# taylorlu/voicepuppet

Hardware: AMD Instinct MI355X
Metric: PixReferNet G+D step frames/sec @256x256 bs=32 (higher is better)
Workload: dtype bf16; 1 GPU; PixReferNet G+D training step (G + 3xD + VGG16-conv3_3 perceptual + TF-Adam x2), 256x256, ngf=ndf=64, global batch 32 = 32 per GPU; global_batch=32, per_gpu_batch=32, parallelism=dp1

## Files before the change

voicepuppet_amd/csrc/conv_args.h:

```cpp
#pragma once
#include <stddef.h>
#include <stdint.h>

namespace vp {

struct TapTable {
  int8_t dh[16];
  int8_t dw[16];
};

struct PixSrc {
  const void* ptr[2];
  int C[2];
  const float* aff_a[2];
  const float* aff_b[2];
  int act;
  int group_n;
};

enum ConvKernel {
  CK_IGEMM = 0,
  CK_PATCH,
  CK_PATCH2,
  CK_SMALLP,
  CK_S2C64,
  CK_CIN8,
  CK_COUT8,
  CK_DCOUT8,
  CK_COUT4,
  CK_C64,
  CK_PATCH3,
  CK_PATCH4,
  CK_DC256,
  CK_DC64,
};
inline int conv_staging(int k) {
  return k <= CK_S2C64 ? k : (k <= CK_COUT4 ? CK_IGEMM : (k <= CK_PATCH4 ? CK_PATCH : CK_PATCH2));
}

struct IgemmArgs {
  PixSrc x;
  int N, Hin, Win;
  int Cin, log2Cin;
  int cin_mask;
  int cin_real;
  int Hg, Wg;
  int sh, sw;
  int ntaps, nclass;
  TapTable taps[4];
  const void* Wp;
  int Kpad, CoutPad;
  int wp_rows;
  void* Y;
  int y_f32;
  int Cout, ldY;
  int Hof, Wof, os;
  int o0h[4], o0w[4];
  const float* bias;
  int out_act;
  const void* ref;
  const float* ref_a;
  const float* ref_b;
  int ref_act, ref_group_n, accumulate;
  int split_c;
  void* Y2;
  const void* ref2;
  int accumulate2;
  int y2_f32;
  int splitk;
  float* partial;
  int vec_epi;
  int fastk;
  int rowperm;
  int xcd_remap;
  double* bn_part;
  int bn_tpg, bn_nchunk;
  const void* bst_y;
  const void* bst_y2;
  double* bn_part2;
  double* colsum_part;
  const void* zeros;
  int kern, p_kw, p_dhf, p_dhs, p_dwf, p_dws;
  void* xa_lrelu;
  void* xa_relu;
  void* pool_out;
  int pool_only;
  unsigned char* pool_code;
  int pool_src;
  unsigned* sp_cnt;
  unsigned short sp_mask[4];
  int sp_npt, sp_lcpt;
};

struct WgradArgs {
  PixSrc g;
  int Gc, log2Gc;
  int gc_mask;
  int Hgin, Wgin;
  PixSrc d;
  int Dc;
  int N, Hb, Wb;
  int s, ntaps;
  TapTable taps;
  int Mpad, Dpad;
  int splitk;
  float* partial;
  float* dW;
  int Greal, Dreal, accumulate;
  const void* zeros;
  int lw, lh;
  int fastw;
  int xcd_remap;
  int fast_tr;
};

struct Cout1Args {
  const void* dy;
  int ld_dy;
  const float* w;
  const void* ref;
  int ref_act;
  const void* y;
  double* part;
  void* dx;
  int N, H, W, C, Ho, Wo, ks, pad;
  int groups, rows;
  float* slabs;
  float* dW;
  int pix_per_group, tiles_per_group;
};

}
```

voicepuppet_amd/csrc/conv_ops.h:

```cpp
#pragma once
#include <stdlib.h>
#include <string.h>

#include "launch.h"

namespace vp {

struct ConvGeomX : ConvGeom {
  int CoutT;
};

inline ConvGeomX make_geom(int kind, int ks, int stride, int pad, int N, int Hin, int Win, int Cin, int Cin_real, int Cout) {
  ConvGeomX g;
  g.kind = kind; g.ks = ks; g.stride = stride; g.pad = pad;
  g.N = N; g.Hin = Hin; g.Win = Win;
  if (kind == 0) { g.Hout = (Hin + 2 * pad - ks) / stride + 1; g.Wout = (Win + 2 * pad - ks) / stride + 1; }
  else { g.Hout = 2 * Hin; g.Wout = 2 * Win; }
  g.Cin = Cin; g.Cin_real = Cin_real; g.Cout = Cout;
  g.CoutT = Cout < 8 ? 8 : Cout;
  return g;
}

inline int kc_elems(int is_bf16) { return is_bf16 ? 32 : 16; }

// ... 10 lines not shown
    if (rows % 128 == 0) return 0;
    if (rows % 64 == 0) return 1;
    if (rows <= 16) return 2;
    return rows > 64 ? 0 : 1;
  }
  if (rows <= 64) return 5;
  return P > 16 ? 3 : 4;
}

constexpr int IGEMM_SPLITK_TARGET_DEFAULT = 64;
inline int& igemm_splitk_target_knob() { static int v = IGEMM_SPLITK_TARGET_DEFAULT; return v; }
inline int pick_igemm_splitk(int blocks, int nchunk) {
  const int target = igemm_splitk_target_knob();
  const int cap = plan_misc_knob(1);
  const int minchunk = plan_misc_knob(2);
  if (blocks >= 256 || blocks >= target) return 1;
  int s = (target + blocks - 1) / blocks;
  if (s > nchunk / minchunk) s = nchunk / minchunk;
  if (s > cap) s = cap;
  return s < 1 ? 1 : s;
}

inline void set_single_src(PixSrc& x, const void* p, int C, const float* a, const float* b, int act, int group_n) {
  x.ptr[0] = p; x.ptr[1] = nullptr; x.C[0] = C; x.C[1] = 0;
  x.aff_a[0] = a; x.aff_b[0] = b; x.aff_a[1] = nullptr; x.aff_b[1] = nullptr;
  x.act = act; x.group_n = group_n > 0 ? group_n : (1 << 30);
}

struct LaunchForm {
  bool bias = false, ref = false, xa_lrelu = false, xa_relu = false, x_affine = false;
  bool stats = false;
  int x_act = 0, ref_act = 0;
};

struct IgemmPlan {
  IgemmArgs a;
  int cfg;
  LaunchForm form;
  PackDesc pack;
  size_t pack_elems;
  size_t partial_bytes;
};

struct IgemmPin { int cfg, splitk; };

inline void finish_igemm(IgemmPlan& p, int rows, int is_bf16, const IgemmPin* pin = nullptr) {
  IgemmArgs& a = p.a;
  const int P = a.N * a.Hg * a.Wg;
  a.Kpad = round_up(a.ntaps * a.Cin, kc_elems(is_bf16));
  p.cfg = pick_igemm_cfg(rows, P, a.Kpad);
  if (!is_bf16 && a.ntaps == 1 && p.cfg == 0) {
    const long long b128 = (long long)((P + 127) / 128) * (rows / 128), b64 = 2 * b128;
    if (((b64 + 255) / 256) * 64 < ((b128 + 255) / 256) * 128) p.cfg = 1;
  }
  if (pin) p.cfg = pin->cfg;
  int bc, bp;
  igemm_tile(p.cfg, &bc, &bp);
  a.CoutPad = round_up(rows, bc);
  if (a.ntaps == 1) { a.log2Cin = 30; a.cin_mask = 0x3fffffff; }
  else { a.log2Cin = ilog2(a.Cin); a.cin_mask = a.Cin - 1; }
  const int blocks = ((P + bp - 1) / bp) * (a.CoutPad / bc) * a.nclass;
  a.splitk = pin ? pin->splitk : pick_igemm_splitk(blocks, a.Kpad / kc_elems(is_bf16));
  p.partial_bytes = a.splitk > 1 ? (size_t)a.nclass * a.splitk * P * a.CoutPad * sizeof(float) : 0;
  {
    const bool tc4 = p.cfg == 0 || p.cfg == 1 || p.cfg == 6 || p.cfg == 7 || p.cfg == 8 || p.cfg == 9;
    a.rowperm = (tc4 && rows % 64 == 0) ? 1 : 0;
    p.pack.perm = a.rowperm;
  }
  a.wp_rows = round_up(rows, 128);
  p.pack.rows_pad = a.wp_rows;
  p.pack.Kpad = a.Kpad;
  p.pack.kc = kc_elems(is_bf16);
  p.pack_elems = (size_t)a.nclass * a.wp_rows * a.Kpad;
}

inline int& patch_tiles_knob() { static int v = 7; return v; }
inline int& patch_small_knob() { static int v = 3; return v; }
inline int& patch_longk_knob() { static int v = 1; return v; }
inline int& patch3_knob() { static int v = 1; return v; }
inline int& wgrad_big_knob() { static int v = 1; return v; }
inline int& patch4_knob() { static int v = 1; return v; }
inline int& c64_knob() { static int v = 1; return v; }
inline int& pool_bwd_fused_knob() { static int v = 1; return v; }
inline int& cout1_knob() { static int v = 256; return v; }
inline int& wgrad1_rows_knob() { static int v = 512; return v; }
inline int& dc64_knob() { static int v = 1; return v; }
inline int& s2c64_knob() { static int v = 512; return v; }
inline int& s2c64_pair_knob() { static int v = 1; return v; }
constexpr int PATCH_MIN_BLOCKS_DEFAULT = 192;
inline int& patch_minblk_knob() { static int v = PATCH_MIN_BLOCKS_DEFAULT; return v; }

inline void patch_tile_hw(int bp, int* th, int* tw) { *th = bp == 128 ? 8 : 16; *tw = bp == 512 ? 32 : 16; }
inline int patch_tile_pixels(int bc) {
  const int k = patch_small_knob();
  if (bc == 256) return (k & 2) ? 128 : 256;
  return (k & 1) ? 256 : 512;
}

inline int patch_tile_rows(int rows, int on) {
  if ((on & 1) && rows % 256 == 0) return 256;
  if ((on & 2) && rows % 128 == 0) return 128;
  if ((on & 4) && rows % 64 == 0) return 64;
  return 0;
}

inline bool plan_patch_eligible(const IgemmPlan& p, int rows, int is_bf16, bool single_src, bool any_grid = false) {
  const int on = patch_tiles_knob();
  const int minblk = any_grid ? 0 : patch_minblk_knob();
  const IgemmArgs& a = p.a;
  const int kc = kc_elems(is_bf16);
  if (!on || !single_src || a.nclass != 1 || a.sh != 1 || a.sw != 1 || a.os != 1 || a.ntaps < 9 || a.Cin % kc || a.Cin < kc) return false;
  if (rows % 64 || a.Cout % 8 || a.ldY % 8 || a.Hg < 16 || a.Wg < 16 || a.Hof != a.Hg || a.Wof != a.Wg) return false;
  const bool p4 = patch4_knob() && is_bf16 && a.ntaps == 16 && rows % 128 == 0;
  if (!p4 && patch_longk_knob() && rows >= 512 && rows % 256 == 0 && a.ntaps * a.Cin >= 4096 && (long long)a.N * a.Hg * a.Wg >= 256 * 256) return false;
  const int bc = p4 ? 128 : patch_tile_rows(rows, on);
  if (!bc) return false;
  int th, tw;
  patch_tile_hw(p4 ? 256 : patch_tile_pixels(bc), &th, &tw);
  const long long blocks = (long long)a.N * ((a.Hg + th - 1) / th) * ((a.Wg + tw - 1) / tw) * (rows / bc);
  const long long p4min = (long long)a.ntaps * a.Cin >= 8192 ? 256 : 512;
  if (p4 && !any_grid && patch_minblk_knob() > 1) {
    if (blocks < p4min) return false;
  } else if (blocks < minblk) return false;
  if ((size_t)a.N * a.Hin * a.Win * a.Cin * (is_bf16 ? 2 : 4) >= 0x70000000ull) return false;
  int ks = 0;
  while (ks * ks < a.ntaps) ++ks;
  if (ks * ks != a.ntaps) return false;
  const int sh = a.taps[0].dh[ks] - a.taps[0].dh[0], sw = a.taps[0].dw[1] - a.taps[0].dw[0];
  if ((sh != 1 && sh != -1) || (sw != 1 && sw != -1)) return false;
  for (int t = 0; t < a.ntaps; ++t)
    if (a.taps[0].dh[t] != a.taps[0].dh[0] + (t / ks) * sh || a.taps[0].dw[t] != a.taps[0].dw[0] + (t % ks) * sw) return false;
  return true;
}
inline void plan_make_patch(IgemmPlan& p, int rows, int is_bf16) {
  IgemmArgs& a = p.a;
  const bool p4 = patch4_knob() && is_bf16 && a.ntaps == 16 && rows % 128 == 0;
  const int bc = p4 ? 128 : patch_tile_rows(rows, patch_tiles_knob());
  int ks = 0;
  while (ks * ks < a.ntaps) ++ks;
  a.kern = CK_PATCH; a.p_kw = ks;
  a.p_dhf = a.taps[0].dh[0]; a.p_dwf = a.taps[0].dw[0];
  a.p_dhs = a.taps[0].dh[ks] - a.taps[0].dh[0]; a.p_dws = a.taps[0].dw[1] - a.taps[0].dw[0];
  const int bp = p4 ? 256 : patch_tile_pixels(bc);
  p.cfg = bc == 256 ? (bp == 128 ? 15 : 10) : (bc == 128 ? (bp == 256 ? 13 : 11) : (bp == 256 ? 14 : 12));
  a.CoutPad = round_up(rows, bc);
  a.splitk = 1;
  p.partial_bytes = 0;
  a.rowperm = 1;
  p.pack.perm = 1;
  p.pack.kswap = 1;
}

inline int& patch_xcd_knob() { static int v = 0; return v; }
inline int& patch2_knob() { static int v = 1; return v; }
inline bool plan_patch2_eligible(const IgemmPlan& p, int rows, int is_bf16, int c0, int c1) {
  const IgemmArgs& a = p.a;
  const int kc = kc_elems(is_bf16);
  if (!patch2_knob() || a.nclass != 4 || a.ntaps != 4 || a.os != 2 || a.sh != 1 || a.sw != 1) return false;
  if (c0 + c1 != a.Cin || c0 % (2 * kc) || c1 % (2 * kc) || c0 < 2 * kc) return false;
  if (rows % 64 || rows > 128 || a.Cout % 8 || a.ldY % 8 || a.Hg < 16 || a.Wg < 16 || a.Hof != 2 * a.Hg || a.Wof != 2 * a.Wg) return false;
  const long long blocks = (long long)a.N * ((a.Hg + 15) / 16) * ((a.Wg + 15) / 16) * 4;
  if (blocks < patch_minblk_knob()) return false;
  const size_t cmax = c0 > c1 ? c0 : c1;
  if ((size_t)a.N * a.Hin * a.Win * cmax * (is_bf16 ? 2 : 4) >= 0x70000000ull) return false;
  for (int cls = 0; cls < 4; ++cls)
    for (int t = 0; t < 4; ++t)
// ... 281 lines not shown
```

voicepuppet_amd/csrc/conv_patch3.hip:

```cpp
#include <stdlib.h>
#ifndef VP_P3_NO_NT
#define VP_NT_STORE 1
#endif
#ifndef VP_P3_ABL
#define VP_P3_ABL 0
#endif

#include <utility>

#include "conv_ops.h"
#include "igemm_device.h"
#include "launch.h"
#include "patch_device.h"

namespace vp {

template <typename T, int WC, int WP, int TC, int TP, int TH, int TW, int NSTW, int KW>
using Patch3Geom = PatchGeom<T, WC, WP, TC, TP, TH, TW, KW - 1, NSTW>;

template <typename T, int WC, int WP, int TC, int TP, int TH, int TW, int STATS, int OCC, int NSTW = 3, int KW = 3>
__global__ __launch_bounds__(512, OCC) void igemm_patch3_kernel(const IgemmArgs a) {
  using G = Patch3Geom<T, WC, WP, TC, TP, TH, TW, NSTW, KW>;
  constexpr int E = G::E, KC = G::KC, NW = G::NW, LA = NSTW - 1;
  constexpr int KS2 = KW * KW, TRIP = 2 * KS2;
  static_assert(TRIP % NSTW == 0 && NSTW >= 3, "ring stages");
  constexpr int JA = G::JA, PW = G::PW, JP = G::JP, PBUFB = G::PBUFB, WSTB = G::WSTB, WBASE = G::WBASE;
  static_assert(JP + LA <= KS2, "one patch DMA per tap step, none in the last LA steps of a chunk");
  extern __shared__ __attribute__((aligned(16))) char smem[];

  const int tid = threadIdx.x, lane = tid & 63;
  const int wave = __builtin_amdgcn_readfirstlane(tid >> 6);
  const int c_base = blockIdx.y * G::BC;
  const PatchTile tile = patch_tile_origin<TH, TW>(a, a.xcd_remap);
  const int n = tile.n, y0 = tile.y0, x0 = tile.x0;
  const bool flip = a.p_dhs < 0;
  const int dh0 = flip ? a.p_dhf - (KW - 1) : a.p_dhf, dw0 = flip ? a.p_dwf - (KW - 1) : a.p_dwf;
  const unsigned es = sizeof(T);
  const int C0 = a.x.C[0];
  const int nchunkc = C0 / KC;

  __amdgpu_buffer_rsrc_t rsW = make_rsrc(reinterpret_cast<const T*>(a.Wp), 0xFFFFFFFFu);
  __amdgpu_buffer_rsrc_t rsX = make_rsrc(a.x.ptr[0], (unsigned)((size_t)a.N * a.Hin * a.Win * C0 * es));

  unsigned pvo[JP];
#pragma unroll
  for (int j = 0; j < JP; ++j) {
    const int pp = (wave + NW * j) * 16 + (lane >> 2);
    const int py = pp / PW, px = pp - py * PW;
    const int ih = y0 + dh0 + py, iw = x0 + dw0 + px;
    const bool ok = pp < G::NPATCH && (unsigned)ih < (unsigned)a.Hin && (unsigned)iw < (unsigned)a.Win;
    const int piece = (lane & 3) ^ ((px >> 2) & 3);
    pvo[j] = ok ? (unsigned)((((n * a.Hin + ih) * a.Win + iw) * C0 + piece * E) * es) : DMA_OOB;
  }
  const PatchWeightDma<G> wdma(c_base, wave, lane);
  const unsigned wstep = (unsigned)(a.wp_rows * KC * es);
  auto issue_w = [&](int u, int chunk, int stage) {
    const int tap = flip ? KS2 - 1 - u : u;
    wdma.issue(rsW, (unsigned)(tap * nchunkc + chunk) * wstep, reinterpret_cast<uint4*>(smem + WBASE + stage * WSTB));
  };
  auto issue_p = [&](int chunk, int buf, int j) {
    uint4* lb = reinterpret_cast<uint4*>(smem + buf * PBUFB);
    dma16_buf(rsX, pvo[j], (unsigned)(chunk * KC) * es, lb + (wave + NW * j) * 64);
  };

  const int wc = wave / WP, wpi = wave - wc * WP;
  const int blkA0 = wc * TC, blkB0 = wpi * TP;
  const int fi = lane & 15, fg = lane >> 4;
  const int aaddr = WBASE + (blkA0 * 64 + fi * 4 + (fg ^ rb_swz(fi))) * 16;
  int tb0[KW][TP];
#pragma unroll
  for (int c = 0; c < KW; ++c)
#pragma unroll
    for (int q = 0; q < TP; ++q) {
      constexpr int BPR = TW / 16;
      const int pb = blkB0 + q;
      const int px = (pb % BPR) * 16 + fi + c;
      const int pp = (pb / BPR) * PW + px;
      tb0[c][q] = (pp << 6) + (((fg ^ (px >> 2)) & 3) << 4) + ((fg & 1) << 3);
    }

  f32x4 acc[TC][TP];
#pragma unroll
  for (int i = 0; i < TC; ++i)
#pragma unroll
    for (int j = 0; j < TP; ++j) acc[i][j] = (f32x4){0.f, 0.f, 0.f, 0.f};

#pragma unroll
  for (int j = 0; j < JP; ++j) issue_p(0, 0, j);
#pragma unroll
  for (int d = 0; d < LA; ++d) issue_w(d % KS2, d / KS2, d % NSTW);

  for (int c = 0; c < ((VP_P3_ABL & 16) ? 0 : nchunkc); c += 2) {
    const bool last_pair = c + 2 >= nchunkc;
    auto step = [&](auto uc) {
      constexpr int U = decltype(uc)::value;
      constexpr int cc = U / KS2, u = U % KS2, pr = u / KW, pc = u % KW, stage = U % NSTW;
      constexpr int NPIECE = [] { int n = 0; for (int k = 1; k <= LA; ++k) n += ((U + TRIP - k) % TRIP % KS2) < JP ? 1 : 0; return n; }();
      constexpr int NV = (LA - 1) * JA + NPIECE;
      constexpr int WLAST = (TRIP - 1 - U < LA - 1 ? TRIP - 1 - U : LA - 1);
#if !(VP_P3_ABL & 2)
      if (U + LA - 1 > TRIP - 1 && last_pair) wait_vm<WLAST * JA + NPIECE>();
      else wait_vm<NV>();
#endif
#if !(VP_P3_ABL & 1)
      __builtin_amdgcn_s_barrier();
#endif
      asm volatile("" ::: "memory");
#if !(VP_P3_ABL & 4)
      {
        constexpr int UL = (U + LA) % TRIP;
        if (U + LA < TRIP) issue_w(UL % KS2, c + UL / KS2, (U + LA) % NSTW);
        else if (!last_pair) issue_w(UL % KS2, c + 2 + UL / KS2, (U + LA) % NSTW);
      }
      if constexpr (u < JP) issue_p(c + cc + 1, 1 - cc, u);
#endif
      constexpr int NA = TC == 8 ? 4 : ((TC == 4 && OCC == 4) ? 2 : TC);
      patch_step_mma<T, TC, TP, NA, stage * WSTB, cc * PBUFB + pr * PW * 64, true>(aaddr, tb0[pc], acc);
    };
    static_steps(step, std::make_integer_sequence<int, TRIP>{});
  }
  asm volatile("s_waitcnt vmcnt(0)" ::: "memory");

#ifndef VP_P3_NO_FASTEPI
  constexpr int NPASS16 = G::BC == 64 ? epi_passes16(G::BC, G::BP, WP, G::RINGB) : 0;
#else
  constexpr int NPASS16 = 0;
#endif
  if (!(VP_P3_ABL & 8) || acc[0][0][0] == 1.2345f) staged_epilogue<T, TC, TP, G::BC, G::BP, G::NPASS, G::NT, STATS, NPASS16>(a, PatchTilePix<TW>{a, n, y0, x0}, c_base, blkA0, blkB0, acc, smem, tile.bt, 0);
}

template <typename T, int WC, int WP, int TC, int TP, int TH, int TW, int OCC, int NSTW = 3, int KW = 3>
static hipError_t launch_patch3_t(const IgemmArgs& b, hipStream_t st) {
  auto kern = b.bn_part ? igemm_patch3_kernel<T, WC, WP, TC, TP, TH, TW, 1, OCC, NSTW, KW> : igemm_patch3_kernel<T, WC, WP, TC, TP, TH, TW, 0, OCC, NSTW, KW>;
  if (b.bst_y) {
    if constexpr (KW == 4) kern = igemm_patch3_kernel<T, WC, WP, TC, TP, TH, TW, 2, OCC, NSTW, KW>;
    else return hipErrorInvalidValue;
  }
  return launch_patch_grid<Patch3Geom<T, WC, WP, TC, TP, TH, TW, NSTW, KW>>(kern, b, 1, st);
}

bool patch3_eligible(const IgemmArgs& a, int is_bf16) {
  const int kc = is_bf16 ? 32 : 16;
  return conv_staging(a.kern) == CK_PATCH && a.ntaps == 9 && a.p_kw == 3 && a.p_dhs == a.p_dws && (a.p_dhs == 1 || a.p_dhs == -1) && a.x.C[0] % (2 * kc) == 0 &&
         a.x.C[1] == 0;
}

bool patch4_eligible(const IgemmArgs& a, int is_bf16) {
  return is_bf16 && conv_staging(a.kern) == CK_PATCH && a.ntaps == 16 && a.p_kw == 4 && a.p_dhs == a.p_dws && (a.p_dhs == 1 || a.p_dhs == -1) &&
         a.x.C[0] % 64 == 0 && a.x.C[1] == 0 && a.CoutPad % 128 == 0 && !a.pool_out;
}
hipError_t launch_igemm_patch4(const IgemmArgs& a, hipStream_t st) {
  IgemmArgs b = a;
  b.vec_epi = 1;
  b.xcd_remap = patch_xcd_knob();
  return launch_patch3_t<bf16, 2, 4, 4, 4, 16, 16, 4, 4, 4>(b, st);
}

hipError_t launch_igemm_patch3(const IgemmArgs& a, int is_bf16, int bc, int bp, hipStream_t st) {
  IgemmArgs b = a;
  b.vec_epi = 1;
  b.xcd_remap = patch_xcd_knob();
#define VP_PATCH3_GO(WC, WP, TC, TP, TH, TW, OCC) \
  (is_bf16 ? launch_patch3_t<bf16, WC, WP, TC, TP, TH, TW, OCC>(b, st) : launch_patch3_t<float, WC, WP, TC, TP, TH, TW, OCC>(b, st))
#define VP_PATCH3_GO6(WC, WP, TC, TP, TH, TW, OCC) \
  (is_bf16 ? launch_patch3_t<bf16, WC, WP, TC, TP, TH, TW, OCC, 6>(b, st) : launch_patch3_t<float, WC, WP, TC, TP, TH, TW, OCC, 6>(b, st))
  if (bc == 256) return bp == 128 ? VP_PATCH3_GO(2, 4, 8, 2, 8, 16, 4) : VP_PATCH3_GO(2, 4, 8, 4, 16, 16, 2);
  if (bc == 128) return bp == 512 ? VP_PATCH3_GO(1, 8, 8, 4, 16, 32, 2) : VP_PATCH3_GO(2, 4, 4, 4, 16, 16, 4);
  if (bp == 512) return VP_PATCH3_GO(1, 8, 4, 4, 16, 32, 2);
  return VP_PATCH3_GO6(2, 4, 2, 4, 16, 16, 4);
#undef VP_PATCH3_GO6
#undef VP_PATCH3_GO
}

}
```

voicepuppet_amd/csrc/igemm_device.h:

```cpp
#pragma once
#include "conv_args.h"
#include "vp_common.h"

namespace vp {

__device__ __forceinline__ int rb_swz(int i) { return (0x78 >> ((i >> 1) & 6)) & 3; }

template <typename T, int TC, int TP, int BC, int BP>
__device__ __forceinline__ void mma_chunk_rb(const uint4* __restrict__ ldsA, const uint4* __restrict__ ldsB,
                                             int blkA0, int blkB0, int lane, f32x4 (&acc)[TC][TP]) {
  const int i = lane & 15, g = lane >> 4;
  const int so = i * 4 + (g ^ rb_swz(i));
  uint4 fa[TC], fb[TP];
#pragma unroll
  for (int t = 0; t < TC; ++t) fa[t] = ldsA[(blkA0 + t) * 64 + so];
#pragma unroll
  for (int t = 0; t < TP; ++t) fb[t] = ldsB[(blkB0 + t) * 64 + so];
#pragma unroll
  for (int tc = 0; tc < TC; ++tc)
#pragma unroll
    for (int tp = 0; tp < TP; ++tp) acc[tc][tp] = mma16<T>(fa[tc], fb[tp], acc[tc][tp]);
}

__device__ __forceinline__ void dma16(const void* src, uint4* lds_dst_wave_uniform) {
// ... 31 lines not shown
}

constexpr int epi_passes16(int BC, int BP, int WP, int ring_bytes) {
  for (int np = 1; np <= WP; np *= 2)
    if ((BP / np) * (BC * 2 + 16) + (BP / np) * 8 <= ring_bytes) return np;
  return WP;
}

template <typename T, bool DUAL = false>
__device__ __forceinline__ void epi_store8(const IgemmArgs& a, long long ot, int c0, size_t off, float (&v)[8]) {
  void* Yp = a.Y;
  const void* refp = a.ref;
  int accu = a.accumulate, yf32 = a.y_f32;
  if constexpr (DUAL) {
    if (c0 >= a.split_c) {
      Yp = a.Y2; refp = a.ref2; accu = a.accumulate2; yf32 = a.y2_f32;
      c0 -= a.split_c; off -= (size_t)a.split_c;
    }
  }
  if (a.bias) {
#pragma unroll
    for (int e = 0; e < 8; ++e) v[e] += a.bias[c0 + e];
  }
  if (a.out_act != ACT_NONE) {
#pragma unroll
    for (int e = 0; e < 8; ++e) v[e] = act_apply(a.out_act, v[e]);
  }
  if (refp) {
    float z[8];
    const T* rp = reinterpret_cast<const T*>(refp) + off;
    if (sizeof(T) == 2) Elem<bf16>::unpack(*reinterpret_cast<const uint4*>(rp), z);
    else {
      Elem<float>::unpack(reinterpret_cast<const uint4*>(rp)[0], z);
      Elem<float>::unpack(reinterpret_cast<const uint4*>(rp)[1], z + 4);
    }
    if (a.ref_a) {
      const int goff = (int)(ot & 255) * a.Cout + c0;
#pragma unroll
      for (int e = 0; e < 8; ++e) z[e] = fmaf(a.ref_a[goff + e], z[e], a.ref_b[goff + e]);
    }
#pragma unroll
    for (int e = 0; e < 8; ++e) v[e] *= act_grad(a.ref_act, z[e]);
  }
  if (yf32 || sizeof(T) == 4) {
    float* yp = reinterpret_cast<float*>(Yp) + off;
    if (accu) {
      const float4 e0 = reinterpret_cast<const float4*>(yp)[0], e1 = reinterpret_cast<const float4*>(yp)[1];
      v[0] += e0.x; v[1] += e0.y; v[2] += e0.z; v[3] += e0.w; v[4] += e1.x; v[5] += e1.y; v[6] += e1.z; v[7] += e1.w;
    }
#ifdef VP_NT_STORE
#pragma unroll
    for (int e = 0; e < 8; ++e) __builtin_nontemporal_store(v[e], yp + e);
#else
    reinterpret_cast<float4*>(yp)[0] = make_float4(v[0], v[1], v[2], v[3]);
    reinterpret_cast<float4*>(yp)[1] = make_float4(v[4], v[5], v[6], v[7]);
#endif
  } else {
    bf16* yp = reinterpret_cast<bf16*>(Yp) + off;
    if (accu) {
      float e[8];
      Elem<bf16>::unpack(*reinterpret_cast<const uint4*>(yp), e);
#pragma unroll
      for (int k = 0; k < 8; ++k) v[k] += e[k];
    }
#ifdef VP_NT_STORE
    { const uint4 pk = Elem<bf16>::pack(v); __builtin_nontemporal_store(pk.x, reinterpret_cast<unsigned*>(yp)); __builtin_nontemporal_store(pk.y, reinterpret_cast<unsigned*>(yp) + 1);
      __builtin_nontemporal_store(pk.z, reinterpret_cast<unsigned*>(yp) + 2); __builtin_nontemporal_store(pk.w, reinterpret_cast<unsigned*>(yp) + 3); }
#else
    *reinterpret_cast<uint4*>(yp) = Elem<bf16>::pack(v);
#endif
  }
}


__device__ __forceinline__ unsigned pool_code_of(float v0, float v1, float v2, float v3) {
  unsigned best = 0;
  float m = v0;
  if (v1 > m) { m = v1; best = 1; }
  if (v2 > m) { m = v2; best = 2; }
  if (v3 > m) { m = v3; best = 3; }
  return m > 0.f ? 1u + best : 0u;
}

template <typename T, int TC, int TP, int BC, int BP, int NPASS, int NT, int STATS = 0, int NPASS16 = 0, bool DUAL = false, typename PixFn>
__device__ __forceinline__ void staged_epilogue(const IgemmArgs& a, const PixFn& pixfn, int c_base, int blkA0, int blkB0,
                                                f32x4 (&acc)[TC][TP], char* smem, int pt = 0, int cls = 0) {
  if constexpr (NPASS16 > 0 && sizeof(T) == 2 && STATS == 0) {
    if (!a.ref && !a.accumulate && !a.y_f32 && (a.out_act == ACT_NONE || a.out_act == ACT_RELU)) {
      constexpr int PITCHB = BC * 2 + 16, CGB = BC / 8, RPB = BP / NPASS16;
      static_assert(RPB % (TP * 16) == 0, "a wave's pixel rows must fall into one pass");
      const int tid = threadIdx.x, lane = tid & 63;
      long long* otab = reinterpret_cast<long long*>(smem + RPB * PITCHB);
#pragma unroll
      for (int ps = 0; ps < NPASS16; ++ps) {
        __syncthreads();
        if (tid < RPB) otab[tid] = pixfn(ps * RPB + tid);
        if (blkB0 * 16 >= ps * RPB && blkB0 * 16 < (ps + 1) * RPB) {
#pragma unroll
          for (int tc = 0; tc < TC; ++tc) {
            const int ch = tile_chan0(a.rowperm, blkA0 + tc, lane >> 4);
            float b4[4] = {0.f, 0.f, 0.f, 0.f};
            if (a.bias && c_base + ch < a.Cout) {
#pragma unroll
              for (int e = 0; e < 4; ++e) b4[e] = a.bias[c_base + ch + e];
            }
#pragma unroll
            for (int tp = 0; tp < TP; ++tp) {
              const int row = (blkB0 + tp) * 16 + (lane & 15) - ps * RPB;
              float v[4];
#pragma unroll
              for (int e = 0; e < 4; ++e) {
                v[e] = acc[tc][tp][e];
                if (a.bias) v[e] += b4[e];
                if (a.out_act != ACT_NONE) v[e] = act_apply(a.out_act, v[e]);
              }
              uint2 pk;
              pk.x = Elem<bf16>::pack2(v[0], v[1]); pk.y = Elem<bf16>::pack2(v[2], v[3]);
              *reinterpret_cast<uint2*>(smem + row * PITCHB + ch * 2) = pk;
            }
            __builtin_amdgcn_sched_barrier(0);
          }
        }
        __syncthreads();
        bool store_y = true;
        if constexpr (pix_has_pool<PixFn>::value) store_y = !(a.pool_out != nullptr && a.pool_only);
        if (store_y)
          for (int idx = tid; idx < RPB * CGB; idx += NT) {
            const int p = idx / CGB, cgp = idx - p * CGB;
            const long long ot = otab[p];
            const int c0 = c_base + cgp * 8;
            if (ot < 0 || c0 >= a.Cout) continue;
            const uint4 pk = *reinterpret_cast<const uint4*>(smem + p * PITCHB + cgp * 16);
            unsigned* yp = reinterpret_cast<unsigned*>(reinterpret_cast<bf16*>(a.Y) + (size_t)(ot >> 8) + c0);
#ifdef VP_NT_STORE
            __builtin_nontemporal_store(pk.x, yp); __builtin_nontemporal_store(pk.y, yp + 1);
            __builtin_nontemporal_store(pk.z, yp + 2); __builtin_nontemporal_store(pk.w, yp + 3);
#else
            *reinterpret_cast<uint4*>(yp) = pk;
#endif
          }
        if constexpr (pix_has_pool<PixFn>::value) {
          if (a.pool_out != nullptr) {
            static_assert(RPB % 32 == 0, "a pass must hold whole pairs of tile rows");
            constexpr int PR = RPB / 4;
            for (int idx = tid; idx < PR * CGB; idx += NT) {
              const int pp = idx / CGB, cgp = idx - pp * CGB;
              const int pyl = pp >> 3, pxl = pp & 7;
              const int c0 = c_base + cgp * 8;
              const long long po = pixfn.pool(ps * (RPB / 32) + pyl, pxl);
              if (po < 0 || c0 >= a.Cout) continue;
              const int r00 = pyl * 32 + pxl * 2;
              float m[8];
#pragma unroll
              for (int k = 0; k < 4; ++k) {
                const int rr = r00 + (k >> 1) * 16 + (k & 1);
                float v[8];
                Elem<bf16>::unpack(*reinterpret_cast<const uint4*>(smem + rr * PITCHB + cgp * 16), v);
#pragma unroll
                for (int e = 0; e < 8; ++e) m[e] = k == 0 ? v[e] : fmaxf(m[e], v[e]);
              }
              *reinterpret_cast<uint4*>(reinterpret_cast<bf16*>(a.pool_out) + po + c0) = Elem<bf16>::pack(m);
              if (a.pool_code) {
                float vv[4][8];
#pragma unroll
                for (int k = 0; k < 4; ++k)
                  Elem<bf16>::unpack(*reinterpret_cast<const uint4*>(smem + (r00 + (k >> 1) * 16 + (k & 1)) * PITCHB + cgp * 16), vv[k]);
                unsigned w[2] = {0u, 0u};
#pragma unroll
                for (int e = 0; e < 8; ++e) w[e >> 2] |= pool_code_of(vv[0][e], vv[1][e], vv[2][e], vv[3][e]) << (8 * (e & 3));
                *reinterpret_cast<uint2*>(a.pool_code + po + c0) = make_uint2(w[0], w[1]);
              }
            }
          }
        }
      }
      return;
    }
  }
  constexpr int PITCH = BC * 4 + 16;
  constexpr int CG = BC / 8;
  constexpr int RP = BP / NPASS;
  static_assert(RP % (TP * 16) == 0, "a wave's pixel rows must fall into one pass");
  const int tid = threadIdx.x, lane = tid & 63;
  long long* otab = reinterpret_cast<long long*>(smem + RP * PITCH);
  static_assert(STATS != 1 || NT % BC == 0, "column sums: whole thread groups per channel");
  static_assert(STATS != 2 || NT % CG == 0, "backward sums: a thread keeps one channel group");
  float bsum = 0.f, bsq = 0.f;
  float gs0[STATS == 2 ? 8 : 1], gs1[STATS == 2 ? 8 : 1];
  const T* gy = nullptr;
  if constexpr (STATS == 2) {
    int c0 = c_base + (tid % CG) * 8;
    const void* yb = a.bst_y;
    int ct = a.Cout;
    if constexpr (DUAL) {
      ct = a.split_c;
      if (c0 >= a.split_c) { yb = a.bst_y2; c0 -= a.split_c; }
    }
#pragma unroll
    for (int e = 0; e < 8; ++e) { gs0[e] = 0.f; gs1[e] = 0.f; }
    if (yb && c0 < ct) gy = reinterpret_cast<const T*>(yb);
  }
#pragma unroll
  for (int ps = 0; ps < NPASS; ++ps) {
    __syncthreads();
    if (tid < RP) otab[tid] = pixfn(ps * RP + tid);
    if (blkB0 * 16 >= ps * RP && blkB0 * 16 < (ps + 1) * RP) {
#pragma unroll
      for (int tp = 0; tp < TP; ++tp)
#pragma unroll
        for (int tc = 0; tc < TC; ++tc) {
          const int row = (blkB0 + tp) * 16 + (lane & 15) - ps * RP;
          const int ch = tile_chan0(a.rowperm, blkA0 + tc, lane >> 4);
          *reinterpret_cast<f32x4*>(smem + row * PITCH + ch * 4) = acc[tc][tp];
          __builtin_amdgcn_sched_barrier(0);
        }
    }
    __syncthreads();
    if constexpr (STATS == 1) {
      const int col = tid % BC;
      for (int rr = tid / BC; rr < RP; rr += NT / BC) {
        if (otab[rr] < 0) continue;
        float x = *reinterpret_cast<const float*>(smem + rr * PITCH + col * 4);
        if (sizeof(T) == 2) x = bf16_bits_to_f32(f32_to_bf16_bits(x));
        bsum += x; bsq = fmaf(x, x, bsq);
      }
    }
    bool store_y = true;
    if constexpr (pix_has_pool<PixFn>::value) store_y = !(a.pool_out != nullptr && a.pool_only);
    if (store_y)
    for (int idx = tid; idx < RP * CG; idx += NT) {
      const int p = idx / CG, cgp = idx - p * CG;
      const long long ot = otab[p];
      const int c0 = c_base + cgp * 8;
      if (ot < 0 || c0 >= a.Cout) continue;
      const size_t off = (size_t)(ot >> 8) + c0;
      float v[8];
      {
        const float4 v0 = *reinterpret_cast<const float4*>(smem + p * PITCH + cgp * 32);
        const float4 v1 = *reinterpret_cast<const float4*>(smem + p * PITCH + cgp * 32 + 16);
        v[0] = v0.x; v[1] = v0.y; v[2] = v0.z; v[3] = v0.w; v[4] = v1.x; v[5] = v1.y; v[6] = v1.z; v[7] = v1.w;
      }
      uint4 ry0 = make_uint4(0, 0, 0, 0), ry1 = make_uint4(0, 0, 0, 0);
      if constexpr (STATS == 2) {
        if (gy) {
          size_t yo = off;
          if constexpr (DUAL) { if (c0 >= a.split_c) yo -= (size_t)a.split_c; }
          ry0 = reinterpret_cast<const uint4*>(gy + yo)[0];
          if (sizeof(T) == 4) ry1 = reinterpret_cast<const uint4*>(gy + yo)[1];
        }
      }
      epi_store8<T, DUAL>(a, ot, c0, off, v);
      if constexpr (STATS == 2) {
        if (gy) {
          float fy[8];
          if (sizeof(T) == 2) Elem<bf16>::unpack(ry0, fy);
          else { Elem<float>::unpack(ry0, fy); Elem<float>::unpack(ry1, fy + 4); }
// ... 112 lines not shown
```

voicepuppet_amd/csrc/launch.h:

```cpp
#pragma once
#include <hip/hip_runtime.h>

#include "conv_args.h"
#include "pointwise_args.h"

namespace vp {

hipError_t launch_igemm(const IgemmArgs& a, int is_bf16, int cfg, hipStream_t st);
void igemm_tile(int cfg, int* bc, int* bp);
hipError_t launch_igemm_patch(const IgemmArgs& a, int is_bf16, int bc, int bp, hipStream_t st);
bool patch3_eligible(const IgemmArgs& a, int is_bf16);
hipError_t launch_igemm_patch3(const IgemmArgs& a, int is_bf16, int bc, int bp, hipStream_t st);
bool patch4_eligible(const IgemmArgs& a, int is_bf16);
hipError_t launch_igemm_patch4(const IgemmArgs& a, hipStream_t st);
bool conv_kernel_ok(const IgemmArgs& a, int is_bf16);
const char* conv_kernel_name(int kern);
bool conv_cin8_eligible(const IgemmArgs& a, int is_bf16);
hipError_t launch_conv_cin8(const IgemmArgs& a, hipStream_t st);
bool conv_cout8_eligible(const IgemmArgs& a, int is_bf16);
hipError_t launch_conv_cout8(const IgemmArgs& a, hipStream_t st);
bool conv_dcout8_eligible(const IgemmArgs& a, int is_bf16);
hipError_t launch_conv_dcout8(const IgemmArgs& a, hipStream_t st);
bool conv_cout4_eligible(const IgemmArgs& a, int is_bf16);
hipError_t launch_conv_cout4(const IgemmArgs& a, hipStream_t st);
bool conv_c64_eligible(const IgemmArgs& a, int is_bf16);
hipError_t launch_conv_c64(const IgemmArgs& a, hipStream_t st);
bool conv_dc64_eligible(const IgemmArgs& a, int is_bf16);
hipError_t launch_conv_dc64(const IgemmArgs& a, hipStream_t st);
int conv_dc64_grid(const IgemmArgs& a);
bool conv_dc256_eligible(const IgemmArgs& a, int is_bf16);
int conv_dc256_grid(const IgemmArgs& a);
hipError_t launch_conv_dc256(const IgemmArgs& a, hipStream_t st);
bool conv_s2c64_eligible(const IgemmArgs& a, int is_bf16);
int conv_s2c64_grid(const IgemmArgs& a);
int conv_s2c64_tiles_per_image(const IgemmArgs& a);
hipError_t launch_conv_s2c64(const IgemmArgs& a, hipStream_t st);
bool conv_cout1_bwd_eligible(const Cout1Args& a);
hipError_t launch_conv_cout1_bwd(const Cout1Args& a, hipStream_t st);
bool conv_cout1_wgrad_eligible(const Cout1Args& a);
hipError_t launch_conv_cout1_wgrad(const Cout1Args& a, hipStream_t st);
hipError_t launch_cout1_wgrad_prof(const Cout1Args& a, hipStream_t st);
hipError_t launch_cout1_bwd_prof(const Cout1Args& a, hipStream_t st);
hipError_t launch_igemm_patch2(const IgemmArgs& a, int is_bf16, int bc, int bp, hipStream_t st);
hipError_t launch_igemm_smallp(const IgemmArgs& a, int is_bf16, hipStream_t st);
struct SmallPArgs;
hipError_t launch_smallp(const SmallPArgs& s, int is_bf16, hipStream_t st);
hipError_t launch_smallp_fused(const SmallPArgs& s, int is_bf16, hipStream_t st);
hipError_t launch_wgrad(const WgradArgs& a, int is_bf16, int cfg, hipStream_t st);
bool wgrad_mm_eligible(const WgradArgs& a, int cfg);
hipError_t launch_wgrad_mm(const WgradArgs& a, int cfg, hipStream_t st);
hipError_t launch_wgrad_tr(const WgradArgs& a, hipStream_t st, const char** variant = nullptr, int* tile_cols = nullptr);
void wgrad_tile(int cfg, int* bm, int* bn);

void profile_enable(int on);
void profile_tag(const char* tag);
size_t profile_collect(char* out, size_t cap);

hipError_t launch_pack_weights(const PackDesc* d_descs, int ndesc, const float* master, void* packed, int is_bf16, hipStream_t st);
hipError_t launch_pack_weights_one(const PackDesc& d, const float* master, void* packed, int is_bf16, hipStream_t st);
int bn_nchunk(int Pg, int C, int G, int is_bf16);
hipError_t launch_bn_stats(const BnArgs& a, int is_bf16, hipStream_t st);
hipError_t launch_bn_finalize(const BnArgs& a, hipStream_t st);
bool bn_small(const BnArgs& a);
hipError_t launch_bn_small_fwd(const BnArgs& a, void* out_lrelu, void* out_relu, int is_bf16, hipStream_t st);
hipError_t launch_bn_small_bwd(const BnArgs& a, int is_bf16, hipStream_t st);
hipError_t launch_bn_bwd(const BnArgs& a, int is_bf16, hipStream_t st);
hipError_t launch_bn_bwd_tail(const BnArgs& a, int is_bf16, hipStream_t st);
hipError_t launch_colsum(const BnArgs& a, int creal, float* out, int accumulate, int is_bf16, hipStream_t st);
hipError_t launch_colsum_tail(const BnArgs& a, int creal, float* out, int accumulate, hipStream_t st);
hipError_t launch_act_apply(const void* y, const float* sc, const float* sh, int C, int Pg, size_t npix,
                            void* out_lrelu, void* out_relu, int is_bf16, hipStream_t st);
hipError_t launch_tap_gather(const TapArgs& a, hipStream_t st);
hipError_t launch_tap_spread(const TapArgs& a, int is_bf16, hipStream_t st);
hipError_t launch_frame_pack(const FramePackArgs& a, hipStream_t st);
hipError_t launch_pack_inputs(const PackInputsArgs& a, int is_bf16, hipStream_t st);
int composite_nblocks(int N, int HW);
hipError_t launch_composite_fwd(const CompositeArgs& a, int is_bf16, hipStream_t st);
hipError_t launch_composite_bwd(const CompositeArgs& a, int is_bf16, hipStream_t st);
hipError_t launch_gan_loss(const GanLossArgs& a, int is_bf16, hipStream_t st);
int perceptual_nblocks(size_t half, int is_bf16);
hipError_t launch_perceptual(const PerceptualArgs& a, int is_bf16, hipStream_t st);
hipError_t launch_loss_final(const LossFinalArgs& a, hipStream_t st);
hipError_t launch_maxpool_fwd(const void* x, void* y, int B, int H, int W, int C, int is_bf16, hipStream_t st);
hipError_t launch_maxpool_bwd(const void* x, const void* dy, void* dx, int B, int H, int W, int C, int is_bf16, hipStream_t st);
hipError_t launch_maxpool_bwd_code(const void* code, const void* dy, void* dx, int B, int H, int W, int C, int is_bf16, hipStream_t st);
hipError_t launch_relu_bwd(const void* y, void* d, size_t n, int is_bf16, hipStream_t st);
hipError_t launch_adam(const AdamArgs& a, hipStream_t st);
hipError_t launch_fetch(const FetchArgs& a, hipStream_t st);
hipError_t launch_grad_pack_bf16(const float* src, void* dst, size_t n, hipStream_t st);
hipError_t launch_grad_unpack_bf16(const void* src, float* dst, size_t n, float scale, hipStream_t st);

struct ConvGeom {
  int kind;
  int ks, stride, pad;
  int N, Hin, Win, Hout, Wout;
  int Cin, Cin_real;
  int Cout;
};

inline int ilog2(int v) { int l = 0; while ((1 << l) < v) ++l; return l; }
inline int round_up(int v, int m) { return (v + m - 1) / m * m; }

}
```

voicepuppet_amd/csrc/ops_api.hip:

```cpp
#include <string.h>

#include <string>

#include "conv_ops.h"
#include "errors.h"
#include "audio_args.h"
#include "launch.h"
#include "vp_common.h"

using namespace vp;

namespace {

bool conv_desc_ok(const vp_conv_desc* d) {
  if (!d || d->n < 1 || d->h < 1 || d->w < 1) return false;
  if (d->cin < 8 || (d->cin & (d->cin - 1))) return false;
  if (d->kind == 1 && (d->ksize != 4 || d->stride != 2 || d->pad != 1)) return false;
  if (d->kind != 0 && d->kind != 1) return false;
  if (d->ksize < 1 || d->ksize > 4 || d->stride < 1 || d->stride > 2) return false;
  if (d->kind == 0 && d->stride == 2 && (d->ksize != 4 || d->pad != 1 || (d->h & 1) || (d->w & 1))) return false;
  return d->dtype == VP_F32 || d->dtype == VP_BF16;
}

ConvGeomX geom_of(const vp_conv_desc* d) {
  return make_geom(d->kind, d->ksize, d->stride, d->pad, d->n, d->h, d->w, d->cin, d->cin, d->cout);
}

size_t align256(size_t v) { return (v + 255) & ~(size_t)255; }

const void* zero_page(char* ws, size_t used, hipStream_t st) {
  char* z = ws + align256(used);
  (void)hipMemsetAsync(z, 0, 256, st);
  return z;
}

}

extern "C" {

int vp_pixrefer_pack_frames(const unsigned char* example_frames, const unsigned char* current_frames, const int* crops,
                            int n, int img_size, float* inputs, float* fg_inputs, float* targets, float* masks, void* stream) {
  if (!example_frames || !current_frames || !crops || !inputs || !fg_inputs || !targets || !masks || n < 1 || img_size < 2) {
    set_err("vp_pixrefer_pack_frames: bad argument");
    return VP_ERR_ARG;
  }
  FramePackArgs a;
  a.ex = example_frames; a.cur = current_frames; a.crops = crops;
  a.inputs = inputs; a.fg_inputs = fg_inputs; a.targets = targets; a.masks = masks;
  a.N = n; a.S = img_size;
  VP_HIP_CHECK(launch_frame_pack(a, (hipStream_t)stream));
  return VP_OK;
}

extern "C" void vp_phase_marks_enable(int on);

int vp_tune(const char* key, int value) {
  if (!key) return VP_ERR_ARG;
  const std::string k(key);
  if (k == "patch_tiles") { patch_tiles_knob() = value; return VP_OK; }
  if (k == "patch_min_blocks") { patch_minblk_knob() = value < 0 ? PATCH_MIN_BLOCKS_DEFAULT : value; return VP_OK; }
  if (k == "patch_small_tiles") { patch_small_knob() = value; return VP_OK; }
  if (k == "patch_long_k_on_256") { patch_longk_knob() = value; return VP_OK; }
  if (k == "wgrad_tr") { wgrad_tr_knob() = value; return VP_OK; }
  if (k == "patch3") { patch3_knob() = value; return VP_OK; }
  if (k == "c64") { c64_knob() = value; return VP_OK; }
  if (k == "dc64") { dc64_knob() = value; return VP_OK; }
  if (k == "pool_bwd_fused") { pool_bwd_fused_knob() = value < 0 || value > 4 ? 1 : value; return VP_OK; }
  if (k == "cout1_wgrad_rows" && value > 0) { wgrad1_rows_knob() = value; return VP_OK; }
  if (k == "cout1_bwd") { cout1_knob() = value < 0 ? 256 : value; return VP_OK; }
  if (k == "s2c64") { s2c64_knob() = value; return VP_OK; }
  if (k == "wgrad_big") { wgrad_big_knob() = value; return VP_OK; }
  if (k == "patch4") { patch4_knob() = value; return VP_OK; }
  if (k == "s2c64_pair") { s2c64_pair_knob() = value; return VP_OK; }
  if (k == "bfm_dwproj") { bfm_dwproj_knob() = value; return VP_OK; }
  if (k == "patch2") { patch2_knob() = value; return VP_OK; }
  if (k == "patch_xcd") { patch_xcd_knob() = value; return VP_OK; }
  if (k == "smallp_max_pixels") { smallp_knob() = value; return VP_OK; }
  if (k == "igemm_splitk_target") { igemm_splitk_target_knob() = value < 0 ? IGEMM_SPLITK_TARGET_DEFAULT : value; return VP_OK; }
  if (k == "wgrad_fixed_x10") { wgrad_cost_knob(0) = value; return VP_OK; }
  if (k == "wgrad_slab_tile_x1000") { wgrad_cost_knob(2) = value < 0 ? 150 : value; return VP_OK; }
  if (k == "wgrad_slab_x100") { wgrad_cost_knob(1) = value; return VP_OK; }
  if (k == "smallp_split_target") { plan_misc_knob(0) = value; return VP_OK; }
  if (k == "igemm_splitk_cap") { plan_misc_knob(1) = value; return VP_OK; }
  if (k == "igemm_splitk_minchunk") { plan_misc_knob(2) = value; return VP_OK; }
  if (k == "wgrad_resident_blocks") { plan_misc_knob(3) = value; return VP_OK; }
  if (k == "igemm_small_grid") { igemm_small_grid_knob() = value; return VP_OK; }
  if (k == "thin_blocks_cout8" && value > 0) { thin_blocks_knob(0) = value; return VP_OK; }
  if (k == "thin_blocks_dcout8" && value > 0) { thin_blocks_knob(1) = value; return VP_OK; }
  if (k == "thin_blocks_cout4" && value > 0) { thin_blocks_knob(2) = value; return VP_OK; }
  if (k == "thin_blocks_cin8" && value > 0) { thin_blocks_knob(3) = value; return VP_OK; }
  if (k == "phase_marks") { vp_phase_marks_enable(value); return VP_OK; }
  set_err("vp_tune: unknown key %s", key);
  return VP_ERR_ARG;
}

static unsigned* smallp_counter_page(char* ws, size_t used, const IgemmArgs& a, hipStream_t st) {
  unsigned* c = (unsigned*)(ws + align256(used) + 256);
  (void)hipMemsetAsync(c, 0, (size_t)smallp_counters(a) * sizeof(unsigned), st);
  return c;
}

size_t vp_conv_workspace_bytes(const vp_conv_desc* d) {
  if (!conv_desc_ok(d)) return 0;
  const int bf = d->dtype == VP_BF16, es = bf ? 2 : 4;
  const ConvGeomX g = geom_of(d);
  size_t best = 0;
  {
    IgemmPlan p = plan_fwd(g, 0, bf);
    best = align256(p.pack_elems * es) + p.partial_bytes;
    plan_kernel(p, g.Cout, bf, d->cin, 0, FAM_SMALLP, LaunchForm{});
    if (p.a.kern == CK_SMALLP) {
      const size_t b = align256(p.pack_elems * es) + align256(p.partial_bytes) + 512 + (size_t)smallp_counters(p.a) * sizeof(unsigned);
      if (b > best) best = b;
    }
  }
  if ((d->cout & (d->cout - 1)) == 0 && d->cout >= 8) {
    IgemmPlan p = plan_bwd_data(g, 0, 0, d->cin, d->cin, d->cin, bf);
    size_t b = align256(p.pack_elems * es) + p.partial_bytes;
    if (b > best) best = b;
    plan_kernel(p, d->cin, bf, d->cout, 0, FAM_SMALLP, LaunchForm{});
    if (p.a.kern == CK_SMALLP) {
      b = align256(p.pack_elems * es) + align256(p.partial_bytes) + 512 + (size_t)smallp_counters(p.a) * sizeof(unsigned);
      if (b > best) best = b;
    }
    for (int plain = 0; plain < 2; ++plain) {
      WgradPlan w = plan_wgrad(g, bf, plain != 0);
      if (w.partial_bytes + 512 > best) best = w.partial_bytes + 512;
    }
  }
  return best + 1024;
}

int vp_conv_fwd(const vp_conv_desc* d, const void* x, const float* in_scale, const float* in_shift,
                const float* w, const float* bias, void* y, void* workspace, void* stream) {
  if (!conv_desc_ok(d) || !x || !w || !y || !workspace) { set_err("vp_conv_fwd: bad argument"); return VP_ERR_ARG; }
  const int bf = d->dtype == VP_BF16, es = bf ? 2 : 4;
  hipStream_t st = (hipStream_t)stream;
  const ConvGeomX g = geom_of(d);
  IgemmPlan p = plan_fwd(g, 0, bf);
  p.a.out_act = d->out_act;
  LaunchForm f;
  f.bias = bias != nullptr; f.x_affine = in_scale != nullptr; f.x_act = d->in_act;
  const bool plain = d->in_act == ACT_NONE && !in_scale;
  plan_kernel(p, g.Cout, bf, d->cin, 0, plain ? (FAM_SMALLP | FAM_PATCH | FAM_PATCH2 | (d->out_act == ACT_NONE ? FAM_S2C64 : 0)) : 0, f);
  char* ws = (char*)workspace;
  VP_HIP_CHECK(launch_pack_weights_one(p.pack, w, ws, bf, st));
  IgemmArgs a = p.a;
  set_single_src(a.x, x, d->cin, in_scale, in_shift, d->in_act, 0);
  a.Wp = ws;
  a.partial = (float*)(ws + align256(p.pack_elems * es));
// ... 93 lines not shown
  if (pixels < 1 || c < 8) return 0;
  const int nch = bn_nchunk(pixels, c, 1, dtype == VP_BF16);
  return (size_t)nch * 2 * c * sizeof(double) + 4 * (size_t)c * sizeof(float) + 1024;
}

static bool bn_ok(int pixels, int c, int dtype) {
  const int e = dtype == VP_BF16 ? 8 : 4;
  return pixels >= 1 && c >= e && c % e == 0 && 256 % (c / e) == 0 && (dtype == VP_F32 || dtype == VP_BF16);
}

int vp_bn_stats(const void* y, int pixels, int c, int dtype, const float* gamma, const float* beta, float eps,
                float* scale, float* shift, float* mean, float* rstd, void* workspace, void* stream) {
  if (!bn_ok(pixels, c, dtype) || !y || !gamma || !beta || !scale || !shift || !mean || !rstd || !workspace) {
    set_err("vp_bn_stats: bad argument");
    return VP_ERR_ARG;
  }
  BnArgs b;
  memset(&b, 0, sizeof(b));
  b.y = y; b.C = c; b.G = 1; b.Pg = pixels;
  b.nchunk = bn_nchunk(pixels, c, 1, dtype == VP_BF16);
  b.partial = (double*)workspace;
  b.gamma = gamma; b.beta = beta; b.aff_a = scale; b.aff_b = shift; b.mu = mean; b.rstd = rstd; b.eps = eps;
  VP_HIP_CHECK(launch_bn_stats(b, dtype == VP_BF16, (hipStream_t)stream));
  return VP_OK;
}

int vp_bn_bwd(const void* y, const void* dz, void* dy, int pixels, int c, int dtype, const float* gamma,
              const float* mean, const float* rstd, float* dgamma, float* dbeta, void* workspace, void* stream) {
  if (!bn_ok(pixels, c, dtype) || !y || !dz || !dy || !gamma || !mean || !rstd || !dgamma || !dbeta || !workspace) {
    set_err("vp_bn_bwd: bad argument");
    return VP_ERR_ARG;
  }
  BnArgs b;
  memset(&b, 0, sizeof(b));
  b.y = y; b.dz = dz; b.dy = dy; b.C = c; b.G = 1; b.Pg = pixels;
  b.nchunk = bn_nchunk(pixels, c, 1, dtype == VP_BF16);
  b.partial = (double*)workspace;
  float* f = (float*)((char*)workspace + (size_t)b.nchunk * 2 * c * sizeof(double));
  b.c1 = f; b.c2 = f + c;
  b.gamma = gamma; b.mu = const_cast<float*>(mean); b.rstd = const_cast<float*>(rstd);
  b.dgamma = dgamma; b.dbeta = dbeta;
  VP_HIP_CHECK(launch_bn_bwd(b, dtype == VP_BF16, (hipStream_t)stream));
  return VP_OK;
}


int vp_maxpool2x2_fwd(const void* x, void* y, int n, int h, int w, int c, int dtype, void* stream) {
  const int e = dtype == VP_BF16 ? 8 : 4;
  if (!x || !y || n < 1 || h < 2 || w < 2 || (h & 1) || (w & 1) || c < e || c % e) { set_err("vp_maxpool2x2_fwd: bad argument"); return VP_ERR_ARG; }
  VP_HIP_CHECK(launch_maxpool_fwd(x, y, n, h, w, c, dtype == VP_BF16, (hipStream_t)stream));
  return VP_OK;
}

int vp_maxpool2x2_bwd(const void* x, const void* dy, void* dx, int n, int h, int w, int c, int dtype, void* stream) {
  const int e = dtype == VP_BF16 ? 8 : 4;
  if (!x || !dy || !dx || n < 1 || h < 2 || w < 2 || (h & 1) || (w & 1) || c < e || c % e) { set_err("vp_maxpool2x2_bwd: bad argument"); return VP_ERR_ARG; }
  VP_HIP_CHECK(launch_maxpool_bwd(x, dy, dx, n, h, w, c, dtype == VP_BF16, (hipStream_t)stream));
  return VP_OK;
}

int vp_maxpool2x2_bwd_code(const void* code, const void* dy, void* dx, int n, int h, int w, int c, int dtype, void* stream) {
  const int e = dtype == VP_BF16 ? 8 : 4;
  if (!code || !dy || !dx || n < 1 || h < 2 || w < 2 || (h & 1) || (w & 1) || c < e || c % e) { set_err("vp_maxpool2x2_bwd_code: bad argument"); return VP_ERR_ARG; }
  VP_HIP_CHECK(launch_maxpool_bwd_code(code, dy, dx, n, h, w, c, dtype == VP_BF16, (hipStream_t)stream));
  return VP_OK;
}

int vp_composite_fwd(const float* gen_out4, const float* targets, float* out4, float* outputs, float* outputs_fg, int n, int hw,
                     void* stream) {
  if (!gen_out4 || !targets || !out4 || !outputs || !outputs_fg || n < 1 || hw < 1) { set_err("vp_composite_fwd: bad argument"); return VP_ERR_ARG; }
  CompositeArgs ca;
  memset(&ca, 0, sizeof(ca));
  ca.y4 = gen_out4; ca.targets = targets; ca.o4 = out4; ca.outputs = outputs; ca.outputs_fg = outputs_fg; ca.N = n; ca.HW = hw; ca.train = 0;
  VP_HIP_CHECK(launch_composite_fwd(ca, 0, (hipStream_t)stream));
  return VP_OK;
}

int vp_gan_loss(const float* logits, void* seed_d, void* seed_g, float* predict, float* losses, int m, float gan_weight, int dtype,
                void* stream) {
  if (!logits || !seed_d || !seed_g || !predict || !losses || m < 1) { set_err("vp_gan_loss: bad argument"); return VP_ERR_ARG; }
  GanLossArgs ga;
  memset(&ga, 0, sizeof(ga));
  ga.logits = logits; ga.dl_d = seed_d; ga.dl_g = seed_g; ga.predict = predict; ga.losses = losses; ga.M = m; ga.gan_weight = gan_weight;
  VP_HIP_CHECK(launch_gan_loss(ga, dtype == VP_BF16, (hipStream_t)stream));
  return VP_OK;
}

int vp_dwconv7x3_bn_act(const float* x, const float* w, const float* bias, float* y, int b, int h, int wd, int c, void* stream) {
  if (!x || !w || !bias || !y || b < 1 || h < 1 || wd < 1 || c < 4 || (c & 3)) { set_err("vp_dwconv7x3_bn_act: bad argument"); return VP_ERR_ARG; }
  VP_HIP_CHECK(launch_dwconv7x3(x, w, bias, y, 0, b, h, wd, c, (hipStream_t)stream));
  return VP_OK;
}

int vp_dwconv7x3_bn_act_t(const void* x, const float* w, const float* bias, void* y, int dtype, int b, int h, int wd, int c, void* stream) {
  if (!x || !w || !bias || !y || b < 1 || h < 1 || wd < 1 || c < 4 || (c & 3) || (dtype != VP_F32 && dtype != VP_BF16)) {
    set_err("vp_dwconv7x3_bn_act_t: bad argument"); return VP_ERR_ARG;
  }
  VP_HIP_CHECK(launch_dwconv7x3(x, w, bias, y, dtype == VP_BF16, b, h, wd, c, (hipStream_t)stream));
  return VP_OK;
}

int vp_conv_first_fwd(const float* x, const float* w, const float* bias, float* y, int b, int h, int w_in, int cout, void* stream) {
  if (!x || !w || !bias || !y || b < 1 || h < 1 || w_in < 1 || cout < 1) { set_err("vp_conv_first_fwd: bad argument"); return VP_ERR_ARG; }
  int pt, ho, pl, wo;
  same_pad(h, 9, 1, &pt, &ho);
  same_pad(w_in, 5, 2, &pl, &wo);
  VP_HIP_CHECK(launch_conv_first(x, w, bias, y, 0, b, h, w_in, wo, cout, pt, pl, (hipStream_t)stream));
  return VP_OK;
}

static IgemmPlan dwproj_pack_plan(int pixels, int ce, int cout) {
  IgemmPlan p = plan_fwd(make_geom(0, 1, 1, 0, 1, pixels, 1, ce, ce, cout), 0, 0);
  p.pack.s_ch = cout;
  p.pack.dst_off = 0;
  p.pack.perm = 0; p.a.rowperm = 0;
  return p;
}

size_t vp_dwproj_workspace_bytes(int ce, int cout) {
  if (ce < 16 || ce % 16 || cout < 1) return 0;
  return align256((size_t)22 * ce * sizeof(float)) + align256(dwproj_pack_plan(1, ce, cout).pack_elems * sizeof(float)) + 256;
}

int vp_dwproj_fwd(const float* ex, const float* w_dw, const float* b_dw, const float* w_proj, const float* b_proj, float* y, int add, int b, int h,
                  int w, int ce, int cout, void* workspace, void* stream) {
  if (!ex || !w_dw || !b_dw || !w_proj || !b_proj || !y || !workspace || b < 1 || h < 1 || w < 1) { set_err("vp_dwproj_fwd: bad argument"); return VP_ERR_ARG; }
  if (!dwproj_eligible(w, ce, cout)) {
    set_err("vp_dwproj_fwd: no kernel for mel width %d, %d expanded and %d output channels (dwproj_eligible)", w, ce, cout);
    return VP_ERR_ARG;
  }
  const size_t ex_bytes = (size_t)b * h * w * ce * sizeof(float);
  if (ex_bytes >= 0xF0000000ull) {
    set_err("vp_dwproj_fwd: the expanded tensor is %zu bytes, the kernel's 32-bit lane offsets stop below 0xF0000000 (%llu)", ex_bytes, 0xF0000000ull);
    return VP_ERR_ARG;
  }
  hipStream_t st = (hipStream_t)stream;
  float* wdw22 = (float*)workspace;
  float* packed = (float*)((char*)workspace + align256((size_t)22 * ce * sizeof(float)));
  VP_HIP_CHECK(hipMemcpyAsync(wdw22, w_dw, (size_t)21 * ce * sizeof(float), hipMemcpyDeviceToDevice, st));
  VP_HIP_CHECK(hipMemcpyAsync(wdw22 + (size_t)21 * ce, b_dw, (size_t)ce * sizeof(float), hipMemcpyDeviceToDevice, st));
  const IgemmPlan p = dwproj_pack_plan(b * h * w, ce, cout);
  VP_HIP_CHECK(launch_pack_weights_one(p.pack, w_proj, packed, 0, st));
  VP_HIP_CHECK(launch_dwproj(ex, wdw22, packed, p.a.wp_rows, b_proj, y, add ? 1 : 0, b, h, w, ce, cout, st));
  return VP_OK;
}

int vp_maxpool_hw(const float* x, float* y, int b, int h, int w, int c, int kh, int kw, int sh, int sw, void* stream) {
  if (!x || !y || b < 1 || h < 1 || w < 1 || c < 4 || (c & 3) || kh < 1 || kw < 1 || sh < 1 || sw < 1) { set_err("vp_maxpool_hw: bad argument"); return VP_ERR_ARG; }
  const int ho = (h + sh - 1) / sh, wo = (w + sw - 1) / sw;
  const int ph = (ho - 1) * sh + kh - h, pw = (wo - 1) * sw + kw - w;
  const int pt = ph > 0 ? ph / 2 : 0, pl = pw > 0 ? pw / 2 : 0;
  VP_HIP_CHECK(launch_maxpool_same(x, y, 0, 0, b, h, w, c, kh, kw, sh, sw, pt, pl, ho, wo, (hipStream_t)stream));
  return VP_OK;
}

int vp_gru_seq(const float* xg, const float* xc, const float* whg, const float* whc, const int* seq_len, float* out, int b, int t,
               void* stream) {
  if (!xg || !xc || !whg || !whc || !seq_len || !out || b < 1 || t < 1) { set_err("vp_gru_seq: bad argument"); return VP_ERR_ARG; }
  VP_HIP_CHECK(launch_gru_seq(xg, xc, whg, whc, seq_len, out, b, t, (hipStream_t)stream));
  return VP_OK;
}

int vp_gru_seq_state(const float* xg, const float* xc, const float* whg, const float* whc, float* hstate, float* out, int b, int t, int t0,
                     int n, void* stream) {
  if (!xg || !xc || !whg || !whc || !hstate || !out || b < 1 || t < 1 || t0 < 0 || n < 0 || t0 + n > t) {
    set_err("vp_gru_seq_state: bad argument"); return VP_ERR_ARG;
  }
// ... 16 lines not shown
```

voicepuppet_amd/csrc/plan_pixrefer.hip:

```cpp
#include <math.h>
#include <stdio.h>
#include <string.h>

#include <mutex>
#include <string>
#include <utility>
#include <vector>

#include "conv_ops.h"
#include "errors.h"
#include "launch.h"
#include "smallp_args.h"
#include "vp_common.h"

namespace vp {

thread_local char g_err[512] = "";
void set_err(const char* fmt, ...) {
  va_list ap;
  va_start(ap, fmt);
  vsnprintf(g_err, sizeof(g_err), fmt, ap);
  va_end(ap);
}

struct Arena {
  char* base;
  size_t off, cap;
  std::vector<std::pair<size_t, size_t>>* track = nullptr;
  void* alloc(size_t bytes) {
    off = (off + 255) & ~(size_t)255;
    void* p = base ? base + off : nullptr;
    if (track) track->push_back({off, bytes});
    off += bytes;
    return p;
  }
};

struct BnBuf {
  float *a, *b, *mu, *rstd, *c1, *c2, *c1g, *c2g;
  double *pb, *pbg;
};

struct Tens {
  std::string name;
  void* y = nullptr;
  void* dz = nullptr;
  int N = 0, H = 0, W = 0, C = 0;
  bool is_f32 = false;
  bool has_bn = false;
  bool is_input = false;
  bool dz_written = false;
  void* dz2 = nullptr;
  bool dz2_written = false;
  void* xa[3] = {nullptr, nullptr, nullptr};
  bool need_act[3] = {false, false, false};
  BnBuf bn{};
  int producer = -1;
  int n_bwd_consumers = 0;
  int dz_writes = 0;
  bool bn_bwd_done = false;
  bool hi = false;
  void* dz32 = nullptr;
  double* cs_part = nullptr;
  int cs_chunks = 0;
  int pb_cap = 0, pbg_cap = 0;
  int bst_chunks = 0, bst_chunks_g = 0;
  size_t elems() const { return (size_t)N * H * W * C; }
};

struct Layer {
  std::string scope;
  ConvGeomX g;
  int src[2] = {-1, -1};
  int nsrc = 1;
  int in_act = ACT_NONE;
  int out_act = ACT_NONE;
  int out = -1;
  bool has_bn = false;
  size_t w_off = 0, b_off = 0, gamma_off = 0, beta_off = 0;
  size_t pk_fwd = 0, pk_bwd[2] = {0, 0}, pk_bwd_alt[2] = {0, 0};
  bool need_bwd[2] = {false, false};
  IgemmPlan fwd, bwd[2], bwd_alt[2];
  IgemmPlan bwd_pair;
  size_t pk_bwd_pair = 0;
  bool has_pair = false;
  IgemmPlan fwd_half;
  size_t pk_fwd_half = 0;
  bool has_fwd_half = false;
  WgradPlan wg;
  size_t desc0 = 0, desc1 = 0;
  bool tapgemm = false;
  bool fwd_stats = false;
  float* tap_S = nullptr;
  void* tap_dyS = nullptr;
  unsigned* sp_cnt_fwd = nullptr;
  unsigned* sp_cnt_bwd[2] = {nullptr, nullptr};
  unsigned* sp_cnt_pair = nullptr;
};

struct ParamInfo { std::string name; size_t off; int ndim; int64_t shape[4]; };

struct Net {
  std::vector<Tens> t;
  std::vector<Layer> l;
  std::vector<ParamInfo> manifest;
  size_t nparams = 0;
  int batch = 0, groups = 1;
  float* params = nullptr;
  float* grads = nullptr;
  char* packed = nullptr;
  size_t packed_elems = 0;
  std::vector<PackDesc> descs;
  PackDesc* d_descs = nullptr;
  unsigned* sp_cnt = nullptr;
  size_t sp_cnt_n = 0;
};

}

using namespace vp;

struct vp_pixrefer {
  vp_pixrefer_desc d;
  int bf16, es;
  Net G, D, V;
  void *gin, *gfg, *din, *vin;
  float *y4, *o4, *outputs, *outputs_fg, *logits, *predict, *losses;
  void *dl_d, *dl_g, *d_din, *d_vin, *dy4, *df3;
  void *vpool1, *vpool2, *d_vpool1, *d_vpool2;
  unsigned char* vpool_code[2];
  bool pool_codes_written;
  bool pool_fuse_ok[2];
  bool pool_bwd_fused;
  bool pool_dz_stale[2];
  double *comp_partial, *perc_partial, *bn_partial;
  char* scratch;
  char* scratch2;
  double* bn_partial2;
  char* scratch3;
  double* bn_partial3;
  char* scratch4;
  double* bn_partial4;
  hipStream_t side, branch;
  hipStream_t branch2;
  hipEvent_t ev_b2join;
  bool use_b2;
  hipEvent_t ev_fork, ev_join, ev_bfork, ev_bjoin;
  hipEvent_t ev_upd_b, ev_upd_m;
  bool overlap, forked;
  int bst_count;
  int bst_on;
  int vgg_fork_layer;
  bool store_first_raw;
  bool ov_on;
  int dfork_point;
  bool dsplit_on;
  hipEvent_t mark[64];
  int nmark;
  bool marks_made;
  int dfork_pending;
  void* zeros;
  size_t scratch_bytes;
  int n_comp, n_perc;
  struct { bool active, d_done; float *m_g, *v_g, *m_d, *v_d; float lr_t_g, lr_t_d, beta1, beta2, eps; } upd;
  int upd_mask;
  bool params_dirty;
  bool vgg_dirty;
  const float *in_targets, *in_masks;
};

namespace vp {

static int add_tensor(Net& n, const std::string& name, int N, int H, int W, int C, bool has_bn, bool is_input) {
  Tens t;
  t.name = name; t.N = N; t.H = H; t.W = W; t.C = C; t.has_bn = has_bn; t.is_input = is_input;
  n.t.push_back(t);
  return (int)n.t.size() - 1;
}

static void add_param(Net& n, const std::string& name, std::initializer_list<int64_t> shape, size_t* off_out) {
  ParamInfo p;
  p.name = name; p.off = n.nparams; p.ndim = (int)shape.size();
  size_t cnt = 1;
  int i = 0;
  for (auto s : shape) { p.shape[i++] = s; cnt *= (size_t)s; }
  for (; i < 4; ++i) p.shape[i] = 1;
  *off_out = n.nparams;
  n.nparams += cnt;
  n.manifest.push_back(p);
}

static int add_layer(Net& n, const std::string& prefix, const std::string& scope, int kind, int ks, int stride, int pad,
                     std::initializer_list<int> srcs, int cin_real, int cout, bool has_bn, int in_act, int out_act,
                     const char* wname, const char* bname) {
  Layer L;
  L.scope = scope;
  L.nsrc = 0;
  int cin = 0;
  for (int s : srcs) {
    L.src[L.nsrc++] = s; cin += n.t[s].C;
    if (in_act != ACT_NONE) n.t[s].need_act[in_act] = true;
  }
  const Tens& t0 = n.t[L.src[0]];
  L.g = make_geom(kind, ks, stride, pad, n.batch, t0.H, t0.W, cin, cin_real, cout);
  L.in_act = in_act; L.out_act = out_act; L.has_bn = has_bn;
  const std::string base = prefix + scope + "/";
  if (kind == 0) add_param(n, base + wname, {ks, ks, cin_real, cout}, &L.w_off);
  else add_param(n, base + wname, {4, 4, cout, cin_real}, &L.w_off);
  add_param(n, base + bname, {cout}, &L.b_off);
  if (has_bn) {
    add_param(n, base + "batch_normalization/gamma", {cout}, &L.gamma_off);
    add_param(n, base + "batch_normalization/beta", {cout}, &L.beta_off);
  }
  L.out = add_tensor(n, scope, n.batch, L.g.Hout, L.g.Wout, L.g.CoutT, has_bn, false);
  n.t[L.out].producer = (int)n.l.size();
  n.l.push_back(L);
  return L.out;
}
// ... 233 lines not shown
    if (training && L.has_pair && L.bwd_pair.a.kern == CK_SMALLP) n.sp_cnt_n += smallp_counters(L.bwd_pair.a);
  }
}

static void carve_net(Net& n, Arena& ar, int es, bool training) {
  for (Tens& t : n.t) {
    if (t.name == "decoder_1" || t.name == "layer_5") {
      continue;
    }
    if (!t.is_input) t.y = ar.alloc(t.elems() * (t.hi ? sizeof(float) : (size_t)es));
    for (int k = 1; k < 3; ++k) if (t.need_act[k]) t.xa[k] = ar.alloc(t.elems() * es);
    if (t.has_bn) {
      const size_t gc = (size_t)n.groups * t.C * sizeof(float);
      t.bn.a = (float*)ar.alloc(gc); t.bn.b = (float*)ar.alloc(gc);
      t.bn.mu = (float*)ar.alloc(gc); t.bn.rstd = (float*)ar.alloc(gc);
      t.bn.c1 = (float*)ar.alloc(gc); t.bn.c2 = (float*)ar.alloc(gc);
      t.bn.c1g = (float*)ar.alloc(gc); t.bn.c2g = (float*)ar.alloc(gc);
      t.bn.pb = (training && t.pb_cap) ? (double*)ar.alloc((size_t)n.groups * t.pb_cap * 2 * t.C * sizeof(double)) : nullptr;
      t.bn.pbg = (training && t.pbg_cap) ? (double*)ar.alloc((size_t)t.pbg_cap * 2 * t.C * sizeof(double)) : nullptr;
    }
  }
  for (Layer& L : n.l) {
    if (!L.tapgemm) continue;
    const size_t q = (size_t)L.g.N * L.g.Hin * L.g.Win * 16;
    L.tap_S = (float*)ar.alloc(q * sizeof(float));
    L.tap_dyS = ar.alloc(q * es);
  }
  n.packed = (char*)ar.alloc(n.packed_elems * es);
  n.d_descs = (PackDesc*)ar.alloc(n.descs.size() * sizeof(PackDesc));
  n.sp_cnt = (unsigned*)ar.alloc((n.sp_cnt_n + 1) * sizeof(unsigned));
  {
    unsigned* c = n.sp_cnt;
    for (Layer& L : n.l) {
      if (L.fwd.a.kern == CK_SMALLP) { L.sp_cnt_fwd = c; c += c ? smallp_counters(L.fwd.a) : 0; }
      for (int s = 0; s < L.nsrc && training; ++s)
        if (L.need_bwd[s] && L.bwd[s].a.kern == CK_SMALLP) { L.sp_cnt_bwd[s] = c; c += c ? smallp_counters(L.bwd[s].a) : 0; }
      if (training && L.has_pair && L.bwd_pair.a.kern == CK_SMALLP) { L.sp_cnt_pair = c; c += c ? smallp_counters(L.bwd_pair.a) : 0; }
    }
  }
}

static size_t carve_all(vp_pixrefer* h, char* base, size_t cap, std::vector<std::pair<size_t, size_t>>* track = nullptr) {
  Arena ar{base, 0, cap};
  ar.track = track;
  const vp_pixrefer_desc& d = h->d;
  const int N = d.batch, H = d.height, es = h->es;
  const size_t px = (size_t)N * H * H;
  h->gin = ar.alloc(px * 8 * es);
  h->gfg = ar.alloc(px * 8 * es);
  h->y4 = (float*)ar.alloc(px * 4 * sizeof(float));
  h->o4 = (float*)ar.alloc(px * 4 * sizeof(float));
  h->outputs = (float*)ar.alloc(px * 3 * sizeof(float));
  h->outputs_fg = (float*)ar.alloc(px * 3 * sizeof(float));
  h->losses = (float*)ar.alloc(8 * sizeof(float));
  h->G.t[0].y = h->gin; h->G.t[1].y = h->gfg;
  carve_net(h->G, ar, es, d.training);
  if (d.training) {
    const int hd = H / 8 - 2;
    const size_t M = (size_t)N * hd * hd;
    h->din = ar.alloc(3 * px * 8 * es);
    h->vin = ar.alloc(2 * px * 8 * es);
    h->logits = (float*)ar.alloc(3 * M * sizeof(float));
    h->predict = (float*)ar.alloc(2 * M * sizeof(float));
    h->dl_d = ar.alloc(3 * M * 8 * es);
    h->dl_g = ar.alloc(M * 8 * es);
    h->d_din = ar.alloc(px * 8 * es);
    h->d_vin = ar.alloc(px * 8 * es);
    h->dy4 = ar.alloc(px * 8 * es);
    h->D.t[0].y = h->din; h->V.t[0].y = h->vin;
    carve_net(h->D, ar, es, true);
    carve_net(h->V, ar, es, true);
    for (Tens& t : h->G.t) if (!t.is_input && t.name != "decoder_1") { t.dz = ar.alloc(t.elems() * es); if (t.hi) t.dz32 = ar.alloc(t.elems() * sizeof(float)); }
    for (Tens& t : h->D.t) if (!t.is_input && t.name != "layer_5") { t.dz = ar.alloc(t.elems() * es); t.dz2 = ar.alloc(t.elems() / 3 * es); }
    for (Net* n : {&h->G, &h->D})
      for (Tens& t : n->t) if (h->bf16 && !t.is_input && !t.has_bn && t.C == 64) t.cs_part = (double*)ar.alloc((size_t)512 * 2 * 64 * sizeof(double));
    for (Tens& t : h->V.t) if (!t.is_input) t.dz = ar.alloc(t.elems() / 2 * es);
    for (const Tens& t : h->V.t) {
      if (t.name == "pool1") h->vpool_code[0] = (unsigned char*)ar.alloc(t.elems() / 2);
      if (t.name == "pool2") h->vpool_code[1] = (unsigned char*)ar.alloc(t.elems() / 2);
    }
    h->n_comp = composite_nblocks(N, H * H);
    h->n_perc = perceptual_nblocks((size_t)N * (H / 4) * (H / 4) * 256, h->bf16);
    h->comp_partial = (double*)ar.alloc((size_t)h->n_comp * 2 * sizeof(double));
    h->perc_partial = (double*)ar.alloc((size_t)h->n_perc * sizeof(double));
  }
  h->zeros = ar.alloc(256);
  h->bn_partial = (double*)ar.alloc((size_t)1024 * 2 * 512 * sizeof(double));
  h->scratch = (char*)ar.alloc(h->scratch_bytes);
  if (d.training) {
    h->bn_partial2 = (double*)ar.alloc((size_t)1024 * 2 * 512 * sizeof(double));
    h->scratch2 = (char*)ar.alloc(h->scratch_bytes);
    h->bn_partial3 = (double*)ar.alloc((size_t)1024 * 2 * 512 * sizeof(double));
    h->scratch3 = (char*)ar.alloc(h->scratch_bytes);
    h->bn_partial4 = (double*)ar.alloc((size_t)1024 * 2 * 512 * sizeof(double));
    h->scratch4 = (char*)ar.alloc(h->scratch_bytes);
  }
  return ar.off + 256;
}

static IgemmArgs pool_fused_view(const IgemmPlan& p) {
  static unsigned char set[16] = {};
  IgemmArgs v = launch_view(p, p.form);
  v.pool_code = set;
  v.pool_src = 1;
  return v;
}

static void init_handle(vp_pixrefer* h, const vp_pixrefer_desc* d) {
  h->d = *d;
  h->bf16 = d->dtype == VP_BF16;
  h->es = h->bf16 ? 2 : 4;
  build_generator(h->G, d->batch, d->height, d->ngf, (!d->training && d->per_sample_bn) ? d->batch : 1);
  size_t smax = 0;
  plan_net(h->G, h->bf16, d->training, d->training, 0, &smax);
  if (d->training) {
    build_discriminator(h->D, d->batch, d->height, d->ndf);
    plan_net(h->D, h->bf16, true, true, d->batch, &smax);
    build_vgg(h->V, d->batch, d->height);
    for (Layer& L : h->V.l) L.g.N = 2 * d->batch;
    plan_net(h->V, h->bf16, true, false, d->batch, &smax, true);
    for (const Layer& L : h->V.l) {
      if (L.scope != "conv1/conv1_2" && L.scope != "conv2/conv2_2") continue;
      const int k = L.scope == "conv2/conv2_2", knob = pool_bwd_fused_knob();
      const IgemmArgs& ba = L.bwd_alt[0].a;
      const bool big = !k || (long long)ba.N * (ba.Hg / 4) * (ba.Wg / 16) >= 4096;
      h->pool_fuse_ok[k] = ((knob == 1 && big) || knob == 2 + k || knob == 4) && h->bf16 && conv_kernel_ok(pool_fused_view(L.bwd_alt[0]), h->bf16);
    }
  }
  h->scratch_bytes = smax + 256;
  h->params_dirty = true;
  h->vgg_dirty = true;
}

static bool valid_desc(const vp_pixrefer_desc* d) {
  if (!d) { set_err("pixrefer descriptor: null"); return false; }
  if (d->batch < 1 || d->height < 256 || d->height % 256 != 0) { set_err("pixrefer descriptor: batch %d / height %d (height must be a multiple of 256)", d->batch, d->height); return false; }
  if (d->ngf < 8 || (d->ngf & (d->ngf - 1)) || d->ndf < 8 || (d->ndf & (d->ndf - 1))) { set_err("pixrefer descriptor: ngf %d / ndf %d must be powers of two >= 8", d->ngf, d->ndf); return false; }
  if (d->ngf > 64 || d->ndf > 64) { set_err("pixrefer descriptor: ngf %d / ndf %d > 64 exceed the batch-norm workspace (512 channels)", d->ngf, d->ndf); return false; }
  if (!d->training && d->per_sample_bn && d->batch > 1024) { set_err("pixrefer descriptor: per-sample batch-norm supports at most 1024 frames per call (got %d)", d->batch); return false; }
  if (d->dtype != VP_F32 && d->dtype != VP_BF16) { set_err("pixrefer descriptor: dtype %d", d->dtype); return false; }
  if ((d->streams != 0 && d->streams != 1 && d->streams != 3 && d->streams != 4) || d->d_backward_fork < 0 || d->d_backward_fork > 3 || d->d_beside_vgg < 0 ||
      d->d_beside_vgg > 2) {
    set_err("pixrefer descriptor: schedule fields streams %d / d_backward_fork %d / d_beside_vgg %d", d->streams, d->d_backward_fork, d->d_beside_vgg);
    return false;
  }
  return true;
}

static void fill_src(const Net& n, const Layer& L, PixSrc& x, int group_n, int sample0, int group0, int es) {
  for (int s = 0; s < 2; ++s) {
    x.ptr[s] = nullptr; x.C[s] = 0; x.aff_a[s] = nullptr; x.aff_b[s] = nullptr;
  }
  for (int s = 0; s < L.nsrc; ++s) {
    const Tens& t = n.t[L.src[s]];
    const void* base = (L.in_act != ACT_NONE) ? t.xa[L.in_act] : t.y;
    x.ptr[s] = (const char*)base + (size_t)sample0 * t.H * t.W * t.C * es;
    x.C[s] = t.C;
  }
  x.act = ACT_NONE;
  x.group_n = group_n;
  (void)group0;
}

static int run_pack(vp_pixrefer* h, Net& n, hipStream_t st) {
  if (n.descs.empty()) return VP_OK;
  VP_HIP_CHECK(launch_pack_weights(n.d_descs, (int)n.descs.size(), n.params, n.packed, h->bf16, st));
  return VP_OK;
}

static char* scratch_of(vp_pixrefer* h, int ss) { return ss == 3 ? h->scratch4 : ss == 2 ? h->scratch3 : ss == 1 ? h->scratch2 : h->scratch; }
static double* bnp_of(vp_pixrefer* h, int ss) { return ss == 3 ? h->bn_partial4 : ss == 2 ? h->bn_partial3 : ss == 1 ? h->bn_partial2 : h->bn_partial; }

static int run_bn_stats(vp_pixrefer* h, Net& n, Layer& L, int fused_chunks, hipStream_t st, int ss = 0) {
  Tens& t = n.t[L.out];
  BnArgs b;
  memset(&b, 0, sizeof(b));
  b.y = t.y; b.C = t.C; b.G = n.groups; b.Pg = (n.batch / n.groups) * t.H * t.W;
  b.nchunk = bn_nchunk(b.Pg, b.C, b.G, h->bf16);
  b.partial = bnp_of(h, ss);
  b.gamma = n.params + L.gamma_off; b.beta = n.params + L.beta_off;
  b.aff_a = t.bn.a; b.aff_b = t.bn.b; b.mu = t.bn.mu; b.rstd = t.bn.rstd;
  b.eps = 1e-5f;
  if (fused_chunks > 0) { b.nchunk = fused_chunks; VP_HIP_CHECK(launch_bn_finalize(b, st)); return VP_OK; }
  if (bn_small(b)) {
    VP_HIP_CHECK(launch_bn_small_fwd(b, t.xa[ACT_LRELU], t.xa[ACT_RELU], h->bf16, st));
    return 1;
  }
  VP_HIP_CHECK(launch_bn_stats(b, h->bf16, st));
  return VP_OK;
}

static bool plan_can_pool(const IgemmPlan& p) {
  if (conv_staging(p.a.kern) != CK_PATCH || (p.a.Hg & 1) || (p.a.Wg & 1)) return false;
  int bc, bp;
  igemm_tile(p.cfg, &bc, &bp);
  int th, tw;
  patch_tile_hw(bp, &th, &tw);
  return tw == 16 && th % 2 == 0;
}

static int epi_stat_chunks(const IgemmPlan& p, int batch, int groups) {
  const IgemmArgs& a = p.a;
  const int fam = conv_staging(a.kern);
  if (a.splitk != 1 || fam == CK_SMALLP || fam == CK_S2C64 || batch % groups) return 0;
  int bc, bp;
  igemm_tile(p.cfg, &bc, &bp);
  const int pg = (batch / groups) * a.Hg * a.Wg;
  if (!(fam || groups == 1 || pg % bp == 0)) return 0;
  int pth = 16, ptw = 16;
  patch_tile_hw(bp, &pth, &ptw);
  const int tpg = fam ? (batch / groups) * ((a.Hg + pth - 1) / pth) * ((a.Wg + ptw - 1) / ptw) : (pg + bp - 1) / bp;
  return a.nclass * tpg;
}

static int run_layer_fwd_half(vp_pixrefer* h, Net& n, Layer& L, int half, hipStream_t st, void* pool_out = nullptr, bool pool_only = false,
                              unsigned char* pool_code = nullptr) {
  IgemmArgs a = L.fwd_half.a;
  a.pool_out = pool_out;
  a.pool_only = pool_out && pool_only ? 1 : 0;
  a.pool_code = a.pool_only ? pool_code : nullptr;
  const int nb = a.N;
  fill_src(n, L, a.x, nb, half * nb, 0, h->es);
  a.Wp = n.packed + L.pk_fwd_half * h->es;
  Tens& to = n.t[L.out];
  a.Y = (char*)to.y + (size_t)half * nb * to.H * to.W * to.C * h->es;
  a.bias = n.params + L.b_off;
  a.partial = nullptr;
  a.zeros = h->zeros;
  profile_tag((L.scope + (half ? ":fwd1" : ":fwd0")).c_str());
  VP_HIP_CHECK(launch_igemm(a, h->bf16, L.fwd_half.cfg, st));
  return VP_OK;
}

static bool first_layer_acts_fused(const vp_pixrefer* h, const Net& n, const Layer& L) {
  return first_layer_shape(h->bf16, n, L) && L.fwd.a.kern == CK_CIN8;
}

static int run_layer_fwd(vp_pixrefer* h, Net& n, Layer& L, hipStream_t st, void* pool_out = nullptr, int ss = 0) {
  IgemmArgs a = L.fwd.a;
  a.pool_out = pool_out;
  fill_src(n, L, a.x, n.batch / n.groups, 0, 0, h->es);
  a.Wp = n.packed + L.pk_fwd * h->es;
  Tens& to = n.t[L.out];
  a.Y = L.tapgemm ? L.tap_S : to.y;
  a.bias = L.has_bn || L.tapgemm ? nullptr : n.params + L.b_off;
  a.partial = (float*)scratch_of(h, ss);
  a.zeros = h->zeros;
  if (a.kern == CK_SMALLP) {
    SmallPArgs sp;
    memset(&sp, 0, sizeof(sp));
    a.sp_cnt = L.sp_cnt_fwd;
    sp.g = a;
    for (int c = 0; c < 4; ++c) sp.tap_mask[c] = a.sp_mask[c];
    sp.slab = a.partial; sp.cnt = a.sp_cnt; sp.part = bnp_of(h, ss);
    sp.mode = L.has_bn ? SP_FWD_BN : SP_PLAIN;
    sp.hi = to.hi ? 1 : 0;
    if (L.has_bn) {
      sp.gamma = n.params + L.gamma_off; sp.beta = n.params + L.beta_off;
      sp.aff_a = to.bn.a; sp.aff_b = to.bn.b; sp.mu = to.bn.mu; sp.rstd = to.bn.rstd;
      sp.out_lrelu = to.need_act[ACT_LRELU] ? to.xa[ACT_LRELU] : nullptr;
      sp.out_relu = to.need_act[ACT_RELU] ? to.xa[ACT_RELU] : nullptr;
      sp.eps = 1e-5f;
    }
    profile_tag((L.scope + ":fwd").c_str());
    VP_HIP_CHECK(launch_smallp_fused(sp, h->bf16, st));
    if (!L.has_bn && (to.need_act[ACT_LRELU] || to.need_act[ACT_RELU]))
      VP_HIP_CHECK(launch_act_apply(to.y, nullptr, nullptr, to.C, (n.batch / n.groups) * to.H * to.W, (size_t)to.N * to.H * to.W,
                                    to.xa[ACT_LRELU], to.xa[ACT_RELU], h->bf16, st));
    return VP_OK;
  }
  bool fused_stats = false;
  int stat_chunks = 0;
  if (L.has_bn && a.kern == CK_DC256 && n.groups == 1) {
    stat_chunks = 2 * conv_dc256_grid(a);
    a.bn_part = bnp_of(h, ss); a.bn_tpg = 1 << 30; a.bn_nchunk = stat_chunks;
    fused_stats = true;
  } else if (L.has_bn && a.kern == CK_S2C64) {
    const int grid = conv_s2c64_grid(a);
    if ((size_t)n.groups * grid * 2 * to.C <= (size_t)1024 * 2 * 512 && n.groups <= 32) {
      stat_chunks = grid;
      a.bn_part = bnp_of(h, ss); a.bn_tpg = (n.batch / n.groups) * conv_s2c64_tiles_per_image(a); a.bn_nchunk = grid;
      fused_stats = true;
    }
  } else if (L.fwd_stats) {
    stat_chunks = epi_stat_chunks(L.fwd, n.batch, n.groups);
    a.bn_part = bnp_of(h, ss); a.bn_tpg = stat_chunks / a.nclass; a.bn_nchunk = stat_chunks;
    fused_stats = true;
  }
  bool acts_fused = false;
  if (first_layer_acts_fused(h, n, L)) {
    a.xa_lrelu = to.need_act[ACT_LRELU] ? to.xa[ACT_LRELU] : nullptr;
    a.xa_relu = to.need_act[ACT_RELU] ? to.xa[ACT_RELU] : nullptr;
    if (!h->store_first_raw) a.Y = nullptr;
    acts_fused = true;
  }
  profile_tag((L.scope + ":fwd").c_str());
  VP_HIP_CHECK(launch_igemm(a, h->bf16, L.fwd.cfg, st));
  if (L.tapgemm) {
    TapArgs ta;
    memset(&ta, 0, sizeof(ta));
// ... 367 lines not shown
    for (const auto& r : regs)
      if (off >= r.first && off + bytes <= r.first + r.second) return;
    fail("%s: [%zu, +%zu) is not inside a carved region", what, off, bytes);
  };
  const int es = h->es;
  for (Net* n : {&h->G, &h->D, &h->V}) {
    if (n->t.empty()) continue;
    for (const Tens& t : n->t) {
      const std::string nm = t.name;
      if (t.name == "decoder_1" || t.name == "layer_5") continue;
      region_of(t.y, t.elems() * (t.hi ? 4 : es), (nm + ".y").c_str());
      for (int k = 1; k < 3; ++k) if (t.need_act[k]) region_of(t.xa[k], t.elems() * es, (nm + ".xa").c_str());
      if (t.has_bn) {
        const size_t gc = (size_t)n->groups * t.C * sizeof(float);
        for (const float* p : {t.bn.a, t.bn.b, t.bn.mu, t.bn.rstd, t.bn.c1, t.bn.c2, t.bn.c1g, t.bn.c2g}) region_of(p, gc, (nm + ".bn").c_str());
        if (d->training && t.pb_cap) region_of(t.bn.pb, (size_t)n->groups * t.pb_cap * 2 * t.C * sizeof(double), (nm + ".bn.pb").c_str());
        if (d->training && t.pbg_cap) region_of(t.bn.pbg, (size_t)t.pbg_cap * 2 * t.C * sizeof(double), (nm + ".bn.pbg").c_str());
        if ((size_t)n->groups * t.C > (size_t)1024 * 512) fail("%s: %d groups x %d channels exceed the batch-norm partial rows", nm.c_str(), n->groups, t.C);
      }
      if (t.cs_part) region_of(t.cs_part, (size_t)512 * 2 * 64 * sizeof(double), (nm + ".cs_part").c_str());
      if (d->training && !t.is_input) {
        const size_t div = n == &h->V ? 2 : 1;
        region_of(t.dz, t.elems() / div * es, (nm + ".dz").c_str());
        if (t.hi) region_of(t.dz32, t.elems() * 4, (nm + ".dz32").c_str());
        if (n == &h->D) region_of(t.dz2, t.elems() / 3 * es, (nm + ".dz2").c_str());
      }
    }
    region_of(n->packed, n->packed_elems * es, "packed weights");
    region_of(n->d_descs, n->descs.size() * sizeof(PackDesc), "pack descriptors");
    for (const PackDesc& p : n->descs) {
      const size_t pe = (size_t)p.nclass * p.Kpad * p.rows_pad;
      if (p.dst_off + pe > n->packed_elems) fail("pack block [%zu, +%zu) outside the %zu-element packed arena", p.dst_off, pe, n->packed_elems);
      if (p.src_off >= n->nparams) fail("pack source %zu outside the %zu-float parameter arena", p.src_off, n->nparams);
    }
    size_t pend = 0;
    for (const ParamInfo& p : n->manifest) {
      size_t cnt = 1;
      for (int i = 0; i < 4; ++i) cnt *= (size_t)p.shape[i];
      if (p.off != pend) fail("parameter %s at %zu: arena not contiguous (expected %zu)", p.name.c_str(), p.off, pend);
      pend = p.off + cnt;
    }
    if (pend != n->nparams) fail("parameter manifest covers %zu of %zu floats", pend, n->nparams);
    for (const Layer& L : n->l) {
      auto plan_ok = [&](const IgemmPlan& p, const char* what) {
        if (p.partial_bytes > h->scratch_bytes) fail("%s %s: split-K slab %zu > scratch %zu", L.scope.c_str(), what, p.partial_bytes, h->scratch_bytes);
        if (p.a.splitk < 1 || p.a.CoutPad < p.a.Cout) fail("%s %s: splitk %d CoutPad %d", L.scope.c_str(), what, p.a.splitk, p.a.CoutPad);
        if (!conv_kernel_ok(launch_view(p, p.form), h->bf16))
          fail("%s %s: the launch is outside the preconditions of its kernel %s", L.scope.c_str(), what, conv_kernel_name(p.a.kern));
      };
      plan_ok(L.fwd, "fwd");
      if (L.has_fwd_half) plan_ok(L.fwd_half, "fwd_half");
      if (d->training && L.has_pair) plan_ok(L.bwd_pair, "bwd_pair");
      if (d->training)
        for (int s2 = 0; s2 < L.nsrc; ++s2) if (L.need_bwd[s2]) { plan_ok(L.bwd[s2], "bwd"); if (n == &h->D || n == &h->V) plan_ok(L.bwd_alt[s2], "bwd_alt"); }
      if (d->training && n != &h->V && L.wg.partial_bytes > h->scratch_bytes) fail("%s wgrad: slab %zu > scratch %zu", L.scope.c_str(), L.wg.partial_bytes, h->scratch_bytes);
      if (L.tapgemm) { region_of(L.tap_S, (size_t)L.g.N * L.g.Hin * L.g.Win * 16 * 4, "tap_S"); region_of(L.tap_dyS, (size_t)L.g.N * L.g.Hin * L.g.Win * 16 * es, "tap_dyS"); }
    }
  }
  const size_t px = (size_t)d->batch * d->height * d->height;
  region_of(h->gin, px * 8 * es, "gin"); region_of(h->gfg, px * 8 * es, "gfg");
  region_of(h->y4, px * 4 * 4, "y4"); region_of(h->o4, px * 4 * 4, "o4");
  region_of(h->outputs, px * 3 * 4, "outputs"); region_of(h->outputs_fg, px * 3 * 4, "outputs_fg");
  region_of(h->scratch, h->scratch_bytes, "scratch"); region_of(h->bn_partial, (size_t)1024 * 2 * 512 * 8, "bn_partial");
  if (d->training) {
    const int hd = d->height / 8 - 2;
    const size_t M = (size_t)d->batch * hd * hd;
    region_of(h->din, 3 * px * 8 * es, "din"); region_of(h->vin, 2 * px * 8 * es, "vin");
    region_of(h->logits, 3 * M * 4, "logits"); region_of(h->predict, 2 * M * 4, "predict");
    region_of(h->dl_d, 3 * M * 8 * es, "dl_d"); region_of(h->dl_g, M * 8 * es, "dl_g");
    region_of(h->d_din, px * 8 * es, "d_din"); region_of(h->d_vin, px * 8 * es, "d_vin"); region_of(h->dy4, px * 8 * es, "dy4");
    for (const Tens& t : h->V.t) {
      if (t.name == "pool1") region_of(h->vpool_code[0], t.elems() / 2, "pool1 codes");
      if (t.name == "pool2") region_of(h->vpool_code[1], t.elems() / 2, "pool2 codes");
    }
    for (const Layer& L : h->V.l) {
      const int k = L.scope == "conv2/conv2_2";
      if ((L.scope != "conv1/conv1_2" && !k) || !h->pool_fuse_ok[k]) continue;
      const Tens& tp = h->V.t[L.out + 1];
      if (tp.name != (k ? "pool2" : "pool1") || tp.H * 2 != h->V.t[L.out].H || tp.C != h->V.t[L.out].C) fail("%s: the tensor behind it is not its 2x2 pool", L.scope.c_str());
      if (L.bwd_alt[0].a.kern != CK_C64 || !conv_kernel_ok(pool_fused_view(L.bwd_alt[0]), h->bf16)) fail("%s bwd_alt: no pooled-source form of kernel %s", L.scope.c_str(), conv_kernel_name(L.bwd_alt[0].a.kern));
      region_of(tp.dz, tp.elems() / 2 * es, (tp.name + ".dz (pooled-source read)").c_str());
      region_of(h->vpool_code[k], tp.elems() / 2, (tp.name + " codes (pooled-source read)").c_str());
    }
    region_of(h->scratch2, h->scratch_bytes, "scratch2"); region_of(h->scratch3, h->scratch_bytes, "scratch3");
    region_of(h->scratch4, h->scratch_bytes, "scratch4"); region_of(h->bn_partial4, (size_t)1024 * 2 * 512 * 8, "bn_partial4");
    region_of(h->bn_partial2, (size_t)1024 * 2 * 512 * 8, "bn_partial2"); region_of(h->bn_partial3, (size_t)1024 * 2 * 512 * 8, "bn_partial3");
  }
  delete h;
  return rc;
}

struct StreamPool {
  int dev = -1;
  hipStream_t side = nullptr, branch = nullptr, branch2 = nullptr;
};
static StreamPool g_pool;
static std::mutex g_pool_mu;

static int pool_streams(bool want_b2, hipStream_t* side, hipStream_t* branch, hipStream_t* branch2) {
  std::lock_guard<std::mutex> lk(g_pool_mu);
  int dev = 0;
  VP_HIP_CHECK(hipGetDevice(&dev));
  if (g_pool.dev >= 0 && g_pool.dev != dev) { set_err("the step executor's streams were created on device %d, this plan is on device %d (one device per process)", g_pool.dev, dev); return VP_ERR_STATE; }
  if (!g_pool.side) {
    int prio_lo = 0, prio_hi = 0;
    (void)hipDeviceGetStreamPriorityRange(&prio_lo, &prio_hi);
    VP_HIP_CHECK(hipStreamCreateWithPriority(&g_pool.side, hipStreamNonBlocking, prio_lo));
    VP_HIP_CHECK(hipStreamCreateWithFlags(&g_pool.branch, hipStreamNonBlocking));
    g_pool.dev = dev;
  }
  if (want_b2 && !g_pool.branch2) VP_HIP_CHECK(hipStreamCreateWithFlags(&g_pool.branch2, hipStreamNonBlocking));
  if (side) *side = g_pool.side;
  if (branch) *branch = g_pool.branch;
  if (branch2) *branch2 = g_pool.branch2;
  return VP_OK;
}

int vp_reserve_streams(void) { return pool_streams(true, nullptr, nullptr, nullptr); }

void* vp_host_stream(void) {
  hipStream_t b2 = nullptr;
  if (pool_streams(true, nullptr, nullptr, &b2)) return nullptr;
  return (void*)b2;
}

int vp_pixrefer_create(const vp_pixrefer_desc* d, void* workspace, size_t workspace_bytes,
                       float* params_g, float* params_d, const float* params_vgg,
                       float* grads_g, float* grads_d, void* stream, vp_pixrefer_t** out) {
  if (!valid_desc(d) || !workspace || !params_g || !out) { set_err("vp_pixrefer_create: bad argument"); return VP_ERR_ARG; }
  if (d->training && (!params_d || !params_vgg || !grads_g || !grads_d)) { set_err("training needs D/VGG params and grad arenas"); return VP_ERR_ARG; }
  vp_pixrefer* h = new vp_pixrefer{};
  init_handle(h, d);
  const size_t need = carve_all(h, nullptr, 0);
  if (workspace_bytes < need) { set_err("workspace too small: %zu < %zu", workspace_bytes, need); delete h; return VP_ERR_WORKSPACE; }
  carve_all(h, (char*)workspace, workspace_bytes);
  h->G.params = params_g; h->G.grads = grads_g;
  h->D.params = params_d; h->D.grads = grads_d;
  h->V.params = const_cast<float*>(params_vgg);
  for (Tens& t : h->G.t) if (t.name == "decoder_1") { t.y = h->y4; t.dz = h->dy4; }
  hipStream_t st = (hipStream_t)stream;
  VP_HIP_CHECK(hipMemsetAsync(h->zeros, 0, 256, st));
  if (d->training) for (Tens& t : h->D.t) if (t.name == "layer_5") { t.y = h->logits; t.dz = h->dl_d; }
  for (Net* n : {&h->G, &h->D, &h->V}) {
    if (n->descs.empty()) continue;
    VP_HIP_CHECK(hipMemcpyAsync(n->d_descs, n->descs.data(), n->descs.size() * sizeof(PackDesc), hipMemcpyHostToDevice, st));
    VP_HIP_CHECK(hipMemsetAsync(n->sp_cnt, 0, (n->sp_cnt_n + 1) * sizeof(unsigned), st));
  }
  VP_HIP_CHECK(hipStreamSynchronize(st));
  h->overlap = false; h->forked = false;
  h->bst_on = 1; h->vgg_fork_layer = 3;
  h->ov_on = true; h->store_first_raw = false; h->dfork_point = d->d_backward_fork ? d->d_backward_fork - 1 : 2; h->dsplit_on = d->d_beside_vgg != 1;
  if (d->training && d->streams != 1) {
    { const int rc = pool_streams(false, &h->side, &h->branch, &h->branch2); if (rc) { delete h; return rc; } }
    VP_HIP_CHECK(hipEventCreateWithFlags(&h->ev_fork, hipEventDisableTiming));
    VP_HIP_CHECK(hipEventCreateWithFlags(&h->ev_join, hipEventDisableTiming));
    h->use_b2 = d->streams != 3;
    VP_HIP_CHECK(hipEventCreateWithFlags(&h->ev_b2join, hipEventDisableTiming));
    VP_HIP_CHECK(hipEventCreateWithFlags(&h->ev_bfork, hipEventDisableTiming));
    VP_HIP_CHECK(hipEventCreateWithFlags(&h->ev_bjoin, hipEventDisableTiming));
    VP_HIP_CHECK(hipEventCreateWithFlags(&h->ev_upd_b, hipEventDisableTiming));
    VP_HIP_CHECK(hipEventCreateWithFlags(&h->ev_upd_m, hipEventDisableTiming));
    h->overlap = true;
  }
  *out = h;
  return VP_OK;
}
// ... 45 lines not shown
size_t vp_pixrefer_desc_size(void) { return sizeof(vp_pixrefer_desc); }

static int forward_impl(vp_pixrefer_t* h, const float* inputs, const float* fg_inputs, int fg_c, const float* targets, const float* masks, void* stream) {
  if (!h || !inputs || !fg_inputs || !targets) { set_err("vp_pixrefer_forward: null argument"); return VP_ERR_ARG; }
  const vp_pixrefer_desc& d = h->d;
  if (d.training && !masks) { set_err("vp_pixrefer_forward: masks required when training"); return VP_ERR_ARG; }
  hipStream_t st = (hipStream_t)stream;
  const int N = d.batch, H = d.height, bf = h->bf16;
  int rc;
  if (h->params_dirty) {
    if ((rc = run_pack(h, h->G, st))) return rc;
    if (d.training) {
      if ((rc = run_pack(h, h->D, st))) return rc;
      if (h->vgg_dirty) { if ((rc = run_pack(h, h->V, st))) return rc; h->vgg_dirty = false; }
    }
    h->params_dirty = false;
  }
  h->in_targets = targets; h->in_masks = masks;
  PackInputsArgs pi;
  memset(&pi, 0, sizeof(pi));
  pi.inputs = inputs; pi.fg_inputs = fg_inputs; pi.gin = h->gin; pi.gfg = h->gfg; pi.din = h->din; pi.vin = h->vin;
  pi.N = N; pi.HW = H * H; pi.train = d.training; pi.fg_c = fg_c;
  phase_mark(h, st, 0);
  VP_HIP_CHECK(launch_pack_inputs(pi, bf, st));

  bool split_vgg = d.training && h->overlap && h->ov_on;
  if (split_vgg) for (Layer& L : h->V.l) split_vgg = split_vgg && L.has_fwd_half;
  auto vgg_real_half = [&]() -> int {
    VP_HIP_CHECK(hipEventRecord(h->ev_fork, st));
    VP_HIP_CHECK(hipStreamWaitEvent(h->side, h->ev_fork, 0));
    Net& Vs = h->V;
    for (size_t i = 0; i < Vs.l.size(); ++i) {
      Layer& L = Vs.l[i];
      const bool pooled = L.scope == "conv1/conv1_2" || L.scope == "conv2/conv2_2";
      const bool fuse = pooled && plan_can_pool(L.fwd_half);
      if ((rc = run_layer_fwd_half(h, Vs, L, 0, h->side, fuse ? Vs.t[L.out + 1].y : nullptr, true))) return rc;
      if (pooled && !fuse) {
        const Tens& ti = Vs.t[L.out];
        Tens& tp = Vs.t[L.out + 1];
        VP_HIP_CHECK(launch_maxpool_fwd(ti.y, tp.y, N, ti.H, ti.W, ti.C, bf, h->side));
      }
    }
    VP_HIP_CHECK(hipEventRecord(h->ev_join, h->side));
    return VP_OK;
  };
  bool vgg_real_started = false;
  if (split_vgg && h->vgg_fork_layer <= 0) { if ((rc = vgg_real_half())) return rc; vgg_real_started = true; }

  const bool split_enc = d.training && h->overlap && h->ov_on;
  if (split_enc) {
    VP_HIP_CHECK(hipEventRecord(h->ev_bfork, st));
    VP_HIP_CHECK(hipStreamWaitEvent(h->branch, h->ev_bfork, 0));
    for (Layer& L : h->G.l) if (L.scope.rfind("encoder_fg_", 0) == 0) if ((rc = run_layer_fwd(h, h->G, L, h->branch, nullptr, 2))) return rc;
    VP_HIP_CHECK(hipEventRecord(h->ev_bjoin, h->branch));
  }
  for (Layer& L : h->G.l) {
    if (split_enc && L.scope.rfind("encoder_fg_", 0) == 0) continue;
    if (split_enc && L.scope == "merged_encoder_2") VP_HIP_CHECK(hipStreamWaitEvent(st, h->ev_bjoin, 0));
    if (split_vgg && !vgg_real_started && (int)(&L - &h->G.l[0]) >= h->vgg_fork_layer) { if ((rc = vgg_real_half())) return rc; vgg_real_started = true; }
    if (g_phase_detail) phase_mark(h, st, 8 + (int)(&L - &h->G.l[0]));
    if ((rc = run_layer_fwd(h, h->G, L, st))) return rc;
  }

  if (split_vgg && !vgg_real_started) { if ((rc = vgg_real_half())) return rc; vgg_real_started = true; }
  CompositeArgs ca;
  memset(&ca, 0, sizeof(ca));
  ca.y4 = h->y4; ca.targets = targets; ca.masks = masks; ca.o4 = h->o4; ca.outputs = h->outputs; ca.outputs_fg = h->outputs_fg;
  ca.din = h->din; ca.vin = h->vin; ca.partial = h->comp_partial; ca.N = N; ca.HW = H * H; ca.train = d.training;
  VP_HIP_CHECK(launch_composite_fwd(ca, bf, st));
  phase_mark(h, st, 1);
  if (!d.training) return VP_OK;

  const bool split_d = h->overlap && h->ov_on && h->dsplit_on;
  hipStream_t sd = split_d ? h->branch : st;
  const int ssd = split_d ? 2 : 0;
  if (split_d) {
    VP_HIP_CHECK(hipEventRecord(h->ev_bfork, st));
    VP_HIP_CHECK(hipStreamWaitEvent(h->branch, h->ev_bfork, 0));
  }
  for (Layer& L : h->D.l) if ((rc = run_layer_fwd(h, h->D, L, sd, nullptr, ssd))) return rc;
  const int hd = H / 8 - 2;
  GanLossArgs ga;
  memset(&ga, 0, sizeof(ga));
  ga.logits = h->logits; ga.dl_d = h->dl_d; ga.dl_g = h->dl_g; ga.predict = h->predict; ga.losses = h->losses;
  ga.M = N * hd * hd; ga.gan_weight = d.gan_weight;
  VP_HIP_CHECK(launch_gan_loss(ga, bf, sd));
  if (split_d) VP_HIP_CHECK(hipEventRecord(h->ev_bjoin, h->branch));

  Net& V = h->V;
  bool codes = split_vgg && bf && !h->store_first_raw && h->vpool_code[0] && h->vpool_code[1];
  for (Layer& L : V.l)
    if (L.scope == "conv1/conv1_2" || L.scope == "conv2/conv2_2") codes = codes && plan_can_pool(L.fwd_half);
  h->pool_codes_written = codes;
  auto vgg_half = [&](int half, hipStream_t s2) -> int {
    for (size_t i = 0; i < V.l.size(); ++i) {
      Layer& L = V.l[i];
      int rc2;
      const bool pooled = L.scope == "conv1/conv1_2" || L.scope == "conv2/conv2_2";
      const bool fuse = pooled && plan_can_pool(L.fwd_half);
      const Tens& ti = V.t[L.out];
      Tens& tp = V.t[pooled ? L.out + 1 : L.out];
      const size_t oi = (size_t)half * N * ti.H * ti.W * ti.C * h->es, op = (size_t)half * N * tp.H * tp.W * tp.C * h->es;
      const bool code = fuse && codes && half == 1;
      if ((rc2 = run_layer_fwd_half(h, V, L, half, s2, fuse ? (char*)tp.y + op : nullptr, code, code ? h->vpool_code[L.scope == "conv2/conv2_2"] : nullptr))) return rc2;
      if (pooled && !fuse) VP_HIP_CHECK(launch_maxpool_fwd((const char*)ti.y + oi, (char*)tp.y + op, N, ti.H, ti.W, ti.C, bf, s2));
    }
    return VP_OK;
  };
  if (split_vgg) {
    if ((rc = vgg_half(1, st))) return rc;
    VP_HIP_CHECK(hipStreamWaitEvent(st, h->ev_join, 0));
  } else {
    for (size_t i = 0; i < V.l.size(); ++i) {
      Layer& L = V.l[i];
      const bool pooled = L.scope == "conv1/conv1_2" || L.scope == "conv2/conv2_2";
      const bool fuse = pooled && plan_can_pool(L.fwd);
      if ((rc = run_layer_fwd(h, V, L, st, fuse ? V.t[L.out + 1].y : nullptr))) return rc;
      if (pooled && !fuse) {
        const Tens& ti = V.t[L.out];
        Tens& tp = V.t[L.out + 1];
        VP_HIP_CHECK(launch_maxpool_fwd(ti.y, tp.y, ti.N, ti.H, ti.W, ti.C, bf, st));
      }
    }
  }
  const Tens& f3 = V.t.back();
  PerceptualArgs pa;
  memset(&pa, 0, sizeof(pa));
  pa.f3 = f3.y; pa.df3 = f3.dz; pa.partial = h->perc_partial; pa.half = f3.elems() / 2; pa.l1_weight = d.l1_weight;
  VP_HIP_CHECK(launch_perceptual(pa, bf, st));

  if (split_d) VP_HIP_CHECK(hipStreamWaitEvent(st, h->ev_bjoin, 0));
  LossFinalArgs lf;
  memset(&lf, 0, sizeof(lf));
  lf.comp_partial = h->comp_partial; lf.n_comp = h->n_comp; lf.perc_partial = h->perc_partial; lf.n_perc = h->n_perc;
  lf.n_out = (double)N * H * H * 3; lf.n_feat = (double)pa.half; lf.losses = h->losses;
  lf.l1_weight = d.l1_weight; lf.gan_weight = d.gan_weight;
  VP_HIP_CHECK(launch_loss_final(lf, st));
  phase_mark(h, st, 2);
  return VP_OK;
}

static int backward_d_on(vp_pixrefer_t* h, hipStream_t st, bool side);
static int fork_d(vp_pixrefer_t* h, hipStream_t st);

static int update_range(vp_pixrefer_t* h, Net& n, float* m, float* v, float lr_t, size_t off0, size_t off1, int l0, int l1, hipStream_t s) {
  if (off1 > off0) {
    AdamArgs a;
    a.p = n.params + off0; a.g = n.grads + off0; a.m = m + off0; a.v = v + off0; a.n = off1 - off0;
    a.lr_t = lr_t; a.beta1 = h->upd.beta1; a.beta2 = h->upd.beta2; a.eps = h->upd.eps;
    VP_HIP_CHECK(launch_adam(a, s));
  }
  const size_t d0 = n.l[l0].desc0, d1 = n.l[l1].desc1;
  if (d1 > d0) VP_HIP_CHECK(launch_pack_weights(n.d_descs + d0, (int)(d1 - d0), n.params, n.packed, h->bf16, s));
  return VP_OK;
}
static int update_d(vp_pixrefer_t* h, hipStream_t s) {
  h->upd.d_done = true;
  return update_range(h, h->D, h->upd.m_d, h->upd.v_d, h->upd.lr_t_d, 0, h->D.nparams, 0, (int)h->D.l.size() - 1, s);
}

int vp_pixrefer_backward(vp_pixrefer_t* h, void* stream) {
  if (!h || !h->d.training) { set_err("vp_pixrefer_backward: needs a training plan"); return VP_ERR_STATE; }
  hipStream_t st = (hipStream_t)stream;
  if (!h->overlap || !h->ov_on) {
    int rc = vp_pixrefer_backward_d(h, stream);
    if (rc) return rc;
    return vp_pixrefer_backward_g(h, stream);
  }
  int rc;
  h->dfork_pending = h->dfork_point;
  if (h->dfork_pending == 0 && (rc = fork_d(h, st))) { h->dfork_pending = 0; return rc; }
  rc = vp_pixrefer_backward_g(h, stream);
  h->dfork_pending = 0;
  if (rc) return rc;
  VP_HIP_CHECK(hipStreamWaitEvent(st, h->ev_join, 0));
  phase_mark(h, st, 7);
  return VP_OK;
}

static int fork_d(vp_pixrefer_t* h, hipStream_t st) {
  h->dfork_pending = 0;
  VP_HIP_CHECK(hipEventRecord(h->ev_fork, st));
  VP_HIP_CHECK(hipStreamWaitEvent(h->side, h->ev_fork, 0));
  int rc = backward_d_on(h, h->side, true);
  if (rc) return rc;
  if (h->upd.active && h->dfork_point == 2 && (rc = update_d(h, h->side))) return rc;
  VP_HIP_CHECK(hipEventRecord(h->ev_join, h->side));
  return VP_OK;
}

int vp_pixrefer_backward_update(vp_pixrefer_t* h, float* m_g, float* v_g, float* m_d, float* v_d, int step_t_g, int step_t_d,
                                float lr, float beta1, float beta2, float eps, void* stream) {
  if (!h || !h->d.training) { set_err("vp_pixrefer_backward_update: needs a training plan"); return VP_ERR_STATE; }
  if (!m_g || !v_g || !m_d || !v_d || step_t_g < 1 || step_t_d < 1) { set_err("vp_pixrefer_backward_update: bad argument"); return VP_ERR_ARG; }
  auto lr_t = [&](int t) { return (float)((double)lr * sqrt(1.0 - pow((double)beta2, t)) / (1.0 - pow((double)beta1, t))); };
  h->upd.active = true; h->upd.d_done = false;
  h->upd.m_g = m_g; h->upd.v_g = v_g; h->upd.m_d = m_d; h->upd.v_d = v_d;
  h->upd.lr_t_g = lr_t(step_t_g); h->upd.lr_t_d = lr_t(step_t_d); h->upd.beta1 = beta1; h->upd.beta2 = beta2; h->upd.eps = eps;
  int rc = vp_pixrefer_backward(h, stream);
  if (!rc && !h->upd.d_done) rc = update_d(h, (hipStream_t)stream);
  h->upd.active = false;
  if (rc) return rc;
  h->params_dirty = false;
  return VP_OK;
}

int vp_pixrefer_update_bucket(vp_pixrefer_t* h, int which, int bucket, float* m, float* v, int step_t, float lr, float beta1, float beta2,
                              float eps, void* stream) {
  if (!h || !h->d.training || !m || !v || step_t < 1 || which < 0 || which > 1 || bucket < 0 || bucket > (which ? 0 : 2)) {
    set_err("vp_pixrefer_update_bucket: bad argument");
    return VP_ERR_ARG;
  }
  const float lr_t = (float)((double)lr * sqrt(1.0 - pow((double)beta2, step_t)) / (1.0 - pow((double)beta1, step_t)));
  h->upd.beta1 = beta1; h->upd.beta2 = beta2; h->upd.eps = eps;
  int rc;
  if (which == 1) {
    rc = update_range(h, h->D, m, v, lr_t, 0, h->D.nparams, 0, (int)h->D.l.size() - 1, (hipStream_t)stream);
    h->upd_mask |= 8;
  } else {
    Net& G = h->G;
    int i_md5 = -1, i_me2 = -1;
    for (int i = 0; i < (int)G.l.size(); ++i) {
      if (G.l[i].scope == "merged_decoder_5") i_md5 = i;
      if (G.l[i].scope == "merged_encoder_2") i_me2 = i;
    }
    const int l0 = bucket == 0 ? i_md5 : (bucket == 1 ? i_me2 : 0);
    const int l1 = bucket == 0 ? (int)G.l.size() - 1 : (bucket == 1 ? i_md5 - 1 : i_me2 - 1);
    const size_t off0 = G.l[l0].w_off, off1 = l1 + 1 < (int)G.l.size() ? G.l[l1 + 1].w_off : G.nparams;
    rc = update_range(h, G, m, v, lr_t, off0, off1, l0, l1, (hipStream_t)stream);
    h->upd_mask |= 1 << bucket;
  }
  if (rc) return rc;
  if (h->upd_mask == 15) { h->upd_mask = 0; h->params_dirty = false; }
  return VP_OK;
}

int vp_pixrefer_backward_d(vp_pixrefer_t* h, void* stream) {
  if (!h || !h->d.training) { set_err("vp_pixrefer_backward_d: needs a training plan"); return VP_ERR_STATE; }
  return backward_d_on(h, (hipStream_t)stream, false);
}

int vp_pixrefer_backward_d_fork(vp_pixrefer_t* h, void* stream) {
  if (!h || !h->d.training) { set_err("vp_pixrefer_backward_d_fork: needs a training plan"); return VP_ERR_STATE; }
  hipStream_t st = (hipStream_t)stream;
  h->forked = h->overlap && h->ov_on;
  if (!h->forked) return backward_d_on(h, st, false);
  h->dfork_pending = h->dfork_point;
  if (h->dfork_pending == 0) return fork_d(h, st);
  return VP_OK;
}

void* vp_pixrefer_side_stream(vp_pixrefer_t* h) { return (h && h->overlap) ? (void*)h->side : nullptr; }

int vp_pixrefer_use_streams(vp_pixrefer_t* h, int n) {
  if (!h || (n != 3 && n != 4)) { set_err("vp_pixrefer_use_streams: 3 or 4"); return VP_ERR_ARG; }
  h->use_b2 = (n == 4) && h->overlap;
  return VP_OK;
}

int vp_pixrefer_set_option(vp_pixrefer_t* h, const char* key, int value) {
  if (!h || !key) { set_err("vp_pixrefer_set_option: null argument"); return VP_ERR_ARG; }
  const std::string k(key);
  if (k == "overlap") { h->ov_on = value != 0; return VP_OK; }
  if (k == "d_backward_fork") { h->dfork_point = value < 0 ? 0 : (value > 2 ? 2 : value); return VP_OK; }
  if (k == "d_beside_vgg") { h->dsplit_on = value != 0; return VP_OK; }
  if (k == "store_first_raw") { h->store_first_raw = value != 0; return VP_OK; }
  if (k == "bwd_sums_in_epilogue") { h->bst_on = value < 0 ? 0 : (value > 2 ? 2 : value); return VP_OK; }
  if (k == "vgg_real_fork") { h->vgg_fork_layer = value < 0 ? 0 : value; return VP_OK; }
  set_err("vp_pixrefer_set_option: unknown key %s", key);
  return VP_ERR_ARG;
}

long long vp_pixrefer_counter(vp_pixrefer_t* h, const char* key) {
  if (!h || !key) return -1;
  if (std::string(key) == "bwd_sums_launches") return h->bst_count;
  if (std::string(key) == "pool_codes_written") return h->pool_codes_written ? 1 : 0;
  if (std::string(key) == "pool_bwd_fused") return h->pool_bwd_fused ? 1 : 0;
  return -1;
}

int vp_pixrefer_backward_d_join(vp_pixrefer_t* h, void* stream) {
  if (!h || !h->d.training) { set_err("vp_pixrefer_backward_d_join: needs a training plan"); return VP_ERR_STATE; }
  if (h->forked && h->dfork_pending) {
    const int rc = fork_d(h, (hipStream_t)stream);
    if (rc) return rc;
  }
  if (h->forked) VP_HIP_CHECK(hipStreamWaitEvent((hipStream_t)stream, h->ev_join, 0));
  h->forked = false;
  return VP_OK;
}

static int backward_d_on(vp_pixrefer_t* h, hipStream_t st, bool side) {
  const int N = h->d.batch;
  int rc;
  Net& D = h->D;

  for (Tens& t : D.t) { t.dz_written = false; t.bst_chunks = 0; t.cs_chunks = 0; }
  for (int i = (int)D.l.size() - 1; i >= 0; --i) {
    Layer& L = D.l[i];
    Tens& to = D.t[L.out];
    if (L.has_bn) if ((rc = run_bn_bwd(h, D, L, true, 0, 3 * N, 0, 3, st, side ? 1 : 0))) return rc;
    const bool save = L.need_bwd[0];
    if (i == 0) L.need_bwd[0] = false;
    rc = run_layer_bwd(h, D, L, to.dz, true, false, 0, 3 * N, 0, st, side ? 1 : 0);
    L.need_bwd[0] = save;
    if (rc) return rc;
  }

  return VP_OK;
}

int vp_pixrefer_backward_g(vp_pixrefer_t* h, void* stream) { return vp_pixrefer_backward_g_stage(h, -1, stream); }

int vp_pixrefer_backward_g_stages(void) { return 3; }

int vp_pixrefer_backward_g_stage(vp_pixrefer_t* h, int stage, void* stream) {
  if (!h || !h->d.training) { set_err("vp_pixrefer_backward_g: needs a training plan"); return VP_ERR_STATE; }
  if (stage > 2) { set_err("vp_pixrefer_backward_g_stage: stage must be < 3"); return VP_ERR_ARG; }
  hipStream_t st = (hipStream_t)stream;
  const vp_pixrefer_desc& d = h->d;
  const int N = d.batch, H = d.height, bf = h->bf16, es = h->es;
  int rc;
  Net &G = h->G, &D = h->D, &V = h->V;
  int i_md5 = -1, i_me2 = -1;
  for (int i = 0; i < (int)G.l.size(); ++i) {
    if (G.l[i].scope == "merged_decoder_5") i_md5 = i;
    if (G.l[i].scope == "merged_encoder_2") i_me2 = i;
  }
  const int l_hi = stage <= 0 ? (int)G.l.size() - 1 : (stage == 1 ? i_md5 - 1 : i_me2 - 1);
  const int l_lo = stage < 0 ? 0 : (stage == 0 ? i_md5 : (stage == 1 ? i_me2 : 0));
  if (stage <= 0) {
  const bool split_d = h->overlap && h->ov_on && h->dsplit_on;
  hipStream_t sd = split_d ? h->branch : st;
  const int ssd = split_d ? 2 : 0;
  if (split_d) {
    VP_HIP_CHECK(hipEventRecord(h->ev_bfork, st));
    VP_HIP_CHECK(hipStreamWaitEvent(h->branch, h->ev_bfork, 0));
  }
  for (Tens& t : D.t) { t.dz2_written = false; t.bst_chunks_g = 0; }
  for (int i = (int)D.l.size() - 1; i >= 0; --i) {
    Layer& L = D.l[i];
    Tens& to = D.t[L.out];
    if (L.has_bn) if ((rc = run_bn_bwd(h, D, L, false, 2 * N, N, 2, 1, sd, ssd, true))) return rc;
    const void* dy = (i == (int)D.l.size() - 1) ? h->dl_g : to.dz2;
    if ((rc = run_layer_bwd(h, D, L, dy, false, true, 2 * N, N, 2, sd, ssd, true))) return rc;
  }
  if (split_d) VP_HIP_CHECK(hipEventRecord(h->ev_bjoin, h->branch));
  if (h->dfork_pending == 1 && (rc = fork_d(h, st))) return rc;
  for (Tens& t : V.t) t.dz_written = false;
  h->pool_bwd_fused = false;
  h->pool_dz_stale[0] = h->pool_dz_stale[1] = false;
  for (int i = (int)V.l.size() - 1; i >= 0; --i) {
    Layer& L = V.l[i];
    Tens& to = V.t[L.out];
    Tens& ti = V.t[L.src[0]];
    IgemmArgs a = L.bwd_alt[0].a;
    set_single_src(a.x, to.dz, L.g.CoutT, nullptr, nullptr, ACT_NONE, 0);
    const int pk = L.scope == "conv2/conv2_2";
    if ((pk || L.scope == "conv1/conv1_2") && h->pool_dz_stale[pk]) {
      a.x.ptr[0] = V.t[L.out + 1].dz;
// ... 71 lines not shown
      const int l0 = i, l1 = i == i_md5 ? (int)G.l.size() - 1 : (i == i_me2 ? i_md5 - 1 : i_me2 - 1);
      const size_t off0 = G.l[l0].w_off, off1 = l1 + 1 < (int)G.l.size() ? G.l[l1 + 1].w_off : G.nparams;
      hipStream_t su = st;
      const bool on_side = h->overlap && h->ov_on && h->dfork_pending == 0 && h->dfork_point >= 0;
      if (h->overlap && h->ov_on && on_side) {
        VP_HIP_CHECK(hipEventRecord(h->ev_upd_b, h->branch));
        VP_HIP_CHECK(hipEventRecord(h->ev_upd_m, st));
        VP_HIP_CHECK(hipStreamWaitEvent(h->side, h->ev_upd_b, 0));
        VP_HIP_CHECK(hipStreamWaitEvent(h->side, h->ev_upd_m, 0));
        if (b2_used) {
          VP_HIP_CHECK(hipEventRecord(h->ev_b2join, h->branch2));
          VP_HIP_CHECK(hipStreamWaitEvent(h->side, h->ev_b2join, 0));
        }
        su = h->side;
      } else if (h->overlap && h->ov_on) {
        VP_HIP_CHECK(hipEventRecord(h->ev_bfork, st));
        VP_HIP_CHECK(hipStreamWaitEvent(h->branch, h->ev_bfork, 0));
        if (b2_used) {
          VP_HIP_CHECK(hipEventRecord(h->ev_b2join, h->branch2));
          VP_HIP_CHECK(hipStreamWaitEvent(h->branch, h->ev_b2join, 0));
        }
        su = h->branch; forked = true;
      }
      if ((rc = update_range(h, G, h->upd.m_g, h->upd.v_g, h->upd.lr_t_g, off0, off1, l0, l1, su))) return rc;
      if (h->overlap && h->ov_on && on_side) VP_HIP_CHECK(hipEventRecord(h->ev_join, h->side));
    }
  }
  if (forked) {
    if (g_phase_detail && (stage < 0 || stage == 2)) phase_mark(h, st, 60);
    VP_HIP_CHECK(hipEventRecord(h->ev_bjoin, h->branch));
    VP_HIP_CHECK(hipStreamWaitEvent(st, h->ev_bjoin, 0));
    if (b2_used) {
      VP_HIP_CHECK(hipEventRecord(h->ev_b2join, h->branch2));
      VP_HIP_CHECK(hipStreamWaitEvent(st, h->ev_b2join, 0));
    }
  }
  if (stage < 0 || stage == 2) phase_mark(h, st, 6);
  return VP_OK;
}

int vp_profile_enable(int on) { profile_enable(on); return VP_OK; }
size_t vp_profile_collect(char* json, size_t cap) { return profile_collect(json, cap); }

int vp_pixrefer_tensor(vp_pixrefer_t* h, const char* name, void** ptr, int64_t shape[4], int* dtype) {
  if (!h || !name || !ptr) return VP_ERR_ARG;
  const int N = h->d.batch, H = h->d.height;
  auto ret = [&](void* p, int64_t a, int64_t b, int64_t c, int64_t e, int dt) {
    *ptr = p;
    if (shape) { shape[0] = a; shape[1] = b; shape[2] = c; shape[3] = e; }
    if (dtype) *dtype = dt;
    return p ? VP_OK : VP_ERR_STATE;
  };
  const std::string s(name);
  const int cd = h->bf16 ? VP_BF16 : VP_F32;
  if (s == "Outputs_raw") return ret(h->outputs, N, H, H, 3, VP_F32);
  if (s == "Outputs_FG") return ret(h->outputs_fg, N, H, H, 3, VP_F32);
  if (s == "gen_out4") return ret(h->o4, N, H, H, 4, VP_F32);
  if (s == "losses") return ret(h->losses, 8, 1, 1, 1, VP_F32);
  const int hd = H / 8 - 2;
  if (s == "Predict") return ret(h->predict, 2, N, hd, hd, VP_F32);
  if (s == "logits") return ret(h->logits, 3 * N, hd, hd, 1, VP_F32);
  if (s == "d_gen_out4") return ret(h->dy4, N, H, H, 8, cd);
  if (s == "d_din") return ret(h->d_din, N, H, H, 8, cd);
  if (s == "d_vin") return ret(h->d_vin, N, H, H, 8, cd);
  const size_t c = s.find('/');
  if (c == std::string::npos) return VP_ERR_ARG;
  const std::string net = s.substr(0, c);
  std::string rest = s.substr(c + 1);
  Net* n = net == "g" ? &h->G : net == "d" ? &h->D : net == "v" ? &h->V : nullptr;
  if (!n) return VP_ERR_ARG;
  std::string field;
  const size_t k = rest.find(':');
  if (k != std::string::npos) { field = rest.substr(k + 1); rest = rest.substr(0, k); }
  for (Tens& t : n->t) {
    if (t.name != rest) continue;
    if (field.empty() && !h->store_first_raw && t.producer >= 0 && first_layer_acts_fused(h, *n, n->l[t.producer])) {
      set_err("vp_pixrefer_tensor: the raw output of %s is not stored (its kernel writes the consumers' activations); vp_pixrefer_set_option(h, \"store_first_raw\", 1) before the forward pass", s.c_str());
      return VP_ERR_STATE;
    }
    if (field.empty() && n == &h->V && h->pool_codes_written && (t.name == "conv1/conv1_2" || t.name == "conv2/conv2_2")) {
      set_err("vp_pixrefer_tensor: the full-resolution output of %s is not stored (the step keeps its 2x2 max pool and the pool's arg-max codes); vp_pixrefer_set_option(h, \"store_first_raw\", 1) before the forward pass", s.c_str());
      return VP_ERR_STATE;
    }
    if (field.empty()) return ret(t.y, t.N, t.H, t.W, t.is_f32 ? (t.name == "decoder_1" ? 4 : 1) : t.C, (t.is_f32 || t.hi) ? VP_F32 : cd);
    if (field == "dz32") return t.hi ? ret(t.dz32, t.N, t.H, t.W, t.C, VP_F32) : VP_ERR_ARG;
    if (field == "dy" && n == &h->V && (t.name == "conv1/conv1_2" || t.name == "conv2/conv2_2") && h->pool_dz_stale[t.name == "conv2/conv2_2"]) {
      const int k = t.name == "conv2/conv2_2";
      const Tens& tp = n->t[(&t - n->t.data()) + 1];
      VP_HIP_CHECK(hipDeviceSynchronize());
      VP_HIP_CHECK(launch_maxpool_bwd_code(h->vpool_code[k], tp.dz, t.dz, t.N / 2, t.H, t.W, t.C, h->bf16, nullptr));
      VP_HIP_CHECK(hipDeviceSynchronize());
      h->pool_dz_stale[k] = false;
    }
    if (field == "dy") return ret(t.dz, n == &h->V ? t.N / 2 : t.N, t.H, t.W, t.C, cd);
    if (!t.has_bn) return VP_ERR_ARG;
    if (field == "scale") return ret(t.bn.a, n->groups, t.C, 1, 1, VP_F32);
    if (field == "shift") return ret(t.bn.b, n->groups, t.C, 1, 1, VP_F32);
    if (field == "mean") return ret(t.bn.mu, n->groups, t.C, 1, 1, VP_F32);
    if (field == "rstd") return ret(t.bn.rstd, n->groups, t.C, 1, 1, VP_F32);
    return VP_ERR_ARG;
  }
  return VP_ERR_ARG;
}

int vp_pixrefer_fetch(vp_pixrefer_t* h, int what, void* dst, void* stream) {
  if (!h || !dst || what < 0 || what > 3) { set_err("vp_pixrefer_fetch: bad argument"); return VP_ERR_ARG; }
  FetchArgs f;
  memset(&f, 0, sizeof(f));
  f.raw3 = h->outputs; f.fg3 = h->outputs_fg; f.o4 = h->o4; f.dst = dst;
  f.npix = (size_t)h->d.batch * h->d.height * h->d.height;
  f.mode = what;
  if (what == 3 && h->d.training) {
    VP_HIP_CHECK(hipMemcpyAsync(dst, h->outputs_fg, f.npix * 3 * sizeof(float), hipMemcpyDeviceToDevice, (hipStream_t)stream));
    return VP_OK;
  }
  VP_HIP_CHECK(launch_fetch(f, (hipStream_t)stream));
  return VP_OK;
}

int vp_grad_pack_bf16(const float* src, void* dst_bf16, size_t n, void* stream) {
  if (!src || !dst_bf16 || n < 1 || ((uintptr_t)src & 31) || ((uintptr_t)dst_bf16 & 15)) { set_err("vp_grad_pack_bf16: bad argument"); return VP_ERR_ARG; }
  VP_HIP_CHECK(launch_grad_pack_bf16(src, dst_bf16, n, (hipStream_t)stream));
  return VP_OK;
}
int vp_grad_unpack_bf16(const void* src_bf16, float* dst, size_t n, float scale, void* stream) {
  if (!src_bf16 || !dst || n < 1 || ((uintptr_t)dst & 31) || ((uintptr_t)src_bf16 & 15)) { set_err("vp_grad_unpack_bf16: bad argument"); return VP_ERR_ARG; }
  VP_HIP_CHECK(launch_grad_unpack_bf16(src_bf16, dst, n, scale, (hipStream_t)stream));
  return VP_OK;
}

int vp_adam_tf(float* params, const float* grads, float* m, float* v, size_t n, int step_t,
               float lr, float beta1, float beta2, float eps, void* stream) {
  if (!params || !grads || !m || !v || step_t < 1) { set_err("vp_adam_tf: bad argument"); return VP_ERR_ARG; }
  AdamArgs a;
  a.p = params; a.g = grads; a.m = m; a.v = v; a.n = n;
  a.lr_t = (float)((double)lr * sqrt(1.0 - pow((double)beta2, step_t)) / (1.0 - pow((double)beta1, step_t)));
  a.beta1 = beta1; a.beta2 = beta2; a.eps = eps;
  VP_HIP_CHECK(launch_adam(a, (hipStream_t)stream));
  return VP_OK;
}

}
```

voicepuppet_amd/csrc/pointwise.hip:

```cpp
#include "pointwise_args.h"
#include "vp_common.h"

namespace vp {

template <int NV>
__device__ __forceinline__ void block_sum(double (&v)[NV], double* sm ) {
  const int lane = threadIdx.x & 63, wave = threadIdx.x >> 6, nw = blockDim.x >> 6;
#pragma unroll
  for (int i = 0; i < NV; ++i) v[i] = wave_sum(v[i]);
  __syncthreads();
  if (lane == 0)
#pragma unroll
    for (int i = 0; i < NV; ++i) sm[i * 16 + wave] = v[i];
  __syncthreads();
  if (threadIdx.x == 0)
#pragma unroll
    for (int i = 0; i < NV; ++i) {
      double s = 0;
      for (int w = 0; w < nw; ++w) s += sm[i * 16 + w];
      v[i] = s;
    }
}

template <typename T>
// ... 538 lines not shown
      a.fg_inputs[pix * 6 + role * 3 + c] = v[0][c] * v[2][c];
      if (role) { a.targets[pix * 3 + c] = v[0][c]; a.masks[pix * 3 + c] = v[2][c]; }
    }
  }
}

template <typename T>
__global__ __launch_bounds__(256) void composite_fwd_kernel(const CompositeArgs a) {
  const size_t total = (size_t)a.N * a.HW;
  double acc[2] = {0, 0};
  for (size_t i = (size_t)blockIdx.x * 256 + threadIdx.x; i < total; i += (size_t)gridDim.x * 256) {
    const float4 y = reinterpret_cast<const float4*>(a.y4)[i];
    const float o[4] = {tanhf(y.x), tanhf(y.y), tanhf(y.z), tanhf(y.w)};
    reinterpret_cast<float4*>(a.o4)[i] = make_float4(o[0], o[1], o[2], o[3]);
    const float al = (o[3] + 1.f) * 0.5f;
    float ofg[3];
#pragma unroll
    for (int c = 0; c < 3; ++c) {
      const float tg = a.targets[i * 3 + c] * 2.f - 1.f;
      const float out = o[c] * al + tg * (1.f - al);
      ofg[c] = o[c] * al + al - 1.f;
      a.outputs[i * 3 + c] = out;
      a.outputs_fg[i * 3 + c] = ofg[c];
      if (a.train) {
        acc[0] += fabsf(tg - out);
        acc[1] += fabsf(a.masks[i * 3 + c] - al);
      }
    }
    if (a.train) {
      T* d = reinterpret_cast<T*>(a.din) + (2 * total + i) * 8;
      T* v = reinterpret_cast<T*>(a.vin) + (total + i) * 8;
      float head[3];
      if (sizeof(T) == 2) {
        const uint2 h = *reinterpret_cast<const uint2*>(d);
        head[0] = __uint_as_float(h.x << 16); head[1] = __uint_as_float(h.x & 0xffff0000u); head[2] = __uint_as_float(h.y << 16);
      } else {
        const float4 h = *reinterpret_cast<const float4*>(d);
        head[0] = h.x; head[1] = h.y; head[2] = h.z;
      }
      const float fd[8] = {head[0], head[1], head[2], ofg[0], ofg[1], ofg[2], 0.f, 0.f};
      const float fv[8] = {ofg[0], ofg[1], ofg[2], 0.f, 0.f, 0.f, 0.f, 0.f};
      store8<T>(d, fd);
      store8<T>(v, fv);
    }
  }
  if (a.train) {
    __shared__ double sm[64];
    block_sum<2>(acc, sm);
    if (threadIdx.x == 0) { a.partial[blockIdx.x * 2] = acc[0]; a.partial[blockIdx.x * 2 + 1] = acc[1]; }
  }
}

template <typename T>
__global__ __launch_bounds__(256) void composite_bwd_kernel(const CompositeArgs a) {
  const size_t total = (size_t)a.N * a.HW;
  const float s = a.l1_weight / (float)((double)total * 3.0);
  for (size_t i = (size_t)blockIdx.x * 256 + threadIdx.x; i < total; i += (size_t)gridDim.x * 256) {
    const float4 o4 = reinterpret_cast<const float4*>(a.o4)[i];
    const float o[4] = {o4.x, o4.y, o4.z, o4.w};
    const float al = (o[3] + 1.f) * 0.5f;
    const T* dd = reinterpret_cast<const T*>(a.d_din) + i * 8 + 3;
    const T* dv = reinterpret_cast<const T*>(a.d_vin) + i * 8;
    float dout[8] = {0, 0, 0, 0, 0, 0, 0, 0};
    float dal = 0.f;
#pragma unroll
    for (int c = 0; c < 3; ++c) {
      const float tg = a.targets[i * 3 + c] * 2.f - 1.f;
      const float out = a.outputs[i * 3 + c];
      const float df = tg - out, dm = a.masks[i * 3 + c] - al;
      const float d_out = -s * ((df > 0.f) - (df < 0.f));
      const float d_al = -s * ((dm > 0.f) - (dm < 0.f));
      const float d_fg = Elem<T>::ld(dd + c) + Elem<T>::ld(dv + c);
      dout[c] = (d_out + d_fg) * al;
      dal += d_out * (o[c] - tg) + d_fg * (o[c] + 1.f) + d_al;
    }
    dout[3] = dal * 0.5f;
#pragma unroll
    for (int c = 0; c < 4; ++c) dout[c] *= (1.f - o[c] * o[c]);
    store8<T>(reinterpret_cast<T*>(a.dy4) + i * 8, dout);
  }
}

template <typename T>
__global__ __launch_bounds__(1024) void gan_loss_kernel(const GanLossArgs a) {
  const float eps = 1e-12f;
  double acc[2] = {0, 0};
  const float invM = 1.f / (float)a.M;
  T* dld = reinterpret_cast<T*>(a.dl_d);
  T* dlg = reinterpret_cast<T*>(a.dl_g);
  for (int i = threadIdx.x; i < a.M; i += 1024) {
    const float p0 = 1.f / (1.f + expf(-a.logits[i]));
    const float p1 = 1.f / (1.f + expf(-a.logits[a.M + i]));
    const float pf = 1.f / (1.f + expf(-a.logits[2 * a.M + i]));
    const float pr = (p0 + p1) * 0.5f;
    a.predict[i] = pr; a.predict[a.M + i] = pf;
    acc[0] += -(logf(pr + eps) * 2.f + logf(1.f - pf + eps));
    acc[1] += -logf(pf + eps);
    const float dpr = -2.f / (pr + eps) * invM * 0.5f;
    float f[8] = {0, 0, 0, 0, 0, 0, 0, 0};
    f[0] = dpr * p0 * (1.f - p0); store8<T>(dld + (size_t)i * 8, f);
    f[0] = dpr * p1 * (1.f - p1); store8<T>(dld + (size_t)(a.M + i) * 8, f);
    f[0] = 1.f / (1.f - pf + eps) * invM * pf * (1.f - pf); store8<T>(dld + (size_t)(2 * a.M + i) * 8, f);
    f[0] = a.gan_weight * (-1.f / (pf + eps)) * invM * pf * (1.f - pf); store8<T>(dlg + (size_t)i * 8, f);
  }
  __shared__ double sm[64];
  block_sum<2>(acc, sm);
  if (threadIdx.x == 0) { a.losses[0] = (float)(acc[0] / a.M); a.losses[1] = (float)(acc[1] / a.M); }
}

template <typename T>
__global__ __launch_bounds__(256) void perceptual_kernel(const PerceptualArgs a) {
  constexpr int E = Elem<T>::E;
  const T* f = reinterpret_cast<const T*>(a.f3);
  T* df = reinterpret_cast<T*>(a.df3);
  const float s = a.l1_weight / (float)a.half;
  double acc[1] = {0};
  const size_t nv = a.half / E;
  for (size_t i = (size_t)blockIdx.x * 256 + threadIdx.x; i < nv; i += (size_t)gridDim.x * 256) {
    float fa[E], fb[E], d[E];
    Elem<T>::unpack(reinterpret_cast<const uint4*>(f)[i], fa);
    Elem<T>::unpack(reinterpret_cast<const uint4*>(f + a.half)[i], fb);
#pragma unroll
    for (int e = 0; e < E; ++e) {
      const float x = fa[e] - fb[e];
      acc[0] += (double)x * x;
      d[e] = (fb[e] > 0.f) ? -s * x : 0.f;
    }
    reinterpret_cast<uint4*>(df)[i] = Elem<T>::pack(d);
  }
  __shared__ double sm[64];
  block_sum<1>(acc, sm);
  if (threadIdx.x == 0) a.partial[blockIdx.x] = acc[0];
}

__global__ __launch_bounds__(256) void loss_final_kernel(const LossFinalArgs a) {
  double v[3] = {0, 0, 0};
  for (int i = threadIdx.x; i < a.n_comp; i += 256) { v[0] += a.comp_partial[2 * i]; v[1] += a.comp_partial[2 * i + 1]; }
  for (int i = threadIdx.x; i < a.n_perc; i += 256) v[2] += a.perc_partial[i];
  __shared__ double sm[64];
  block_sum<3>(v, sm);
  if (threadIdx.x != 0) return;
  const double content = v[2] / 2.0 / a.n_feat;
  const double gl1 = v[0] / a.n_out + v[1] / a.n_out + content;
  a.losses[2] = (float)gl1;
  a.losses[3] = (float)((double)a.losses[1] * a.gan_weight + gl1 * a.l1_weight);
  a.losses[4] = (float)content;
}

template <typename T>
__global__ __launch_bounds__(256) void maxpool_fwd_kernel(const T* __restrict__ x, T* __restrict__ y, int B, int H, int W, int C) {
  constexpr int E = Elem<T>::E;
  const int ncg = C / E, Ho = H / 2, Wo = W / 2;
  const size_t total = (size_t)B * Ho * Wo * ncg;
  for (size_t i = (size_t)blockIdx.x * 256 + threadIdx.x; i < total; i += (size_t)gridDim.x * 256) {
    const int cg = (int)(i % ncg);
    size_t t = i / ncg;
    const int ow = (int)(t % Wo); t /= Wo;
    const int oh = (int)(t % Ho);
    const int n = (int)(t / Ho);
    const T* p = x + (((size_t)n * H + 2 * oh) * W + 2 * ow) * C + cg * E;
    float m[E], v[E];
    Elem<T>::unpack(*reinterpret_cast<const uint4*>(p), m);
    Elem<T>::unpack(*reinterpret_cast<const uint4*>(p + C), v);
#pragma unroll
    for (int e = 0; e < E; ++e) m[e] = fmaxf(m[e], v[e]);
    Elem<T>::unpack(*reinterpret_cast<const uint4*>(p + (size_t)W * C), v);
#pragma unroll
    for (int e = 0; e < E; ++e) m[e] = fmaxf(m[e], v[e]);
    Elem<T>::unpack(*reinterpret_cast<const uint4*>(p + (size_t)W * C + C), v);
#pragma unroll
    for (int e = 0; e < E; ++e) m[e] = fmaxf(m[e], v[e]);
    *reinterpret_cast<uint4*>(y + i * E) = Elem<T>::pack(m);
  }
}

template <typename T>
__global__ __launch_bounds__(256) void maxpool_bwd_kernel(const T* __restrict__ x, const T* __restrict__ dy, T* __restrict__ dx, int B, int H, int W, int C) {
  constexpr int E = Elem<T>::E;
  const int ncg = C / E, Ho = H / 2, Wo = W / 2;
  const size_t total = (size_t)B * Ho * Wo * ncg;
  for (size_t i = (size_t)blockIdx.x * 256 + threadIdx.x; i < total; i += (size_t)gridDim.x * 256) {
    const int cg = (int)(i % ncg);
    size_t t = i / ncg;
    const int ow = (int)(t % Wo); t /= Wo;
    const int oh = (int)(t % Ho);
    const int n = (int)(t / Ho);
    const size_t base = (((size_t)n * H + 2 * oh) * W + 2 * ow) * C + cg * E;
    const size_t offs[4] = {0, (size_t)C, (size_t)W * C, (size_t)W * C + C};
    float v[4][E], g[E];
#pragma unroll
    for (int k = 0; k < 4; ++k) Elem<T>::unpack(*reinterpret_cast<const uint4*>(x + base + offs[k]), v[k]);
    Elem<T>::unpack(*reinterpret_cast<const uint4*>(dy + i * E), g);
    float o[4][E];
#pragma unroll
    for (int e = 0; e < E; ++e) {
      int best = 0;
      float m = v[0][e];
#pragma unroll
      for (int k = 1; k < 4; ++k) if (v[k][e] > m) { m = v[k][e]; best = k; }
#pragma unroll
      for (int k = 0; k < 4; ++k) o[k][e] = (k == best && m > 0.f) ? g[e] : 0.f;
    }
#pragma unroll
    for (int k = 0; k < 4; ++k) *reinterpret_cast<uint4*>(dx + base + offs[k]) = Elem<T>::pack(o[k]);
  }
}

template <typename T>
__global__ __launch_bounds__(256) void maxpool_bwd_code_kernel(const unsigned char* __restrict__ code, const T* __restrict__ dy, T* __restrict__ dx, int B, int H, int W, int C) {
  constexpr int E = Elem<T>::E;
  const int ncg = C / E, Ho = H / 2, Wo = W / 2;
  const size_t total = (size_t)B * Ho * Wo * ncg;
  for (size_t i = (size_t)blockIdx.x * 256 + threadIdx.x; i < total; i += (size_t)gridDim.x * 256) {
    const int cg = (int)(i % ncg);
    size_t t = i / ncg;
    const int ow = (int)(t % Wo); t /= Wo;
    const int oh = (int)(t % Ho);
    const int n = (int)(t / Ho);
    const size_t base = (((size_t)n * H + 2 * oh) * W + 2 * ow) * C + cg * E;
    const size_t offs[4] = {0, (size_t)C, (size_t)W * C, (size_t)W * C + C};
    unsigned cw[2];
    if constexpr (E == 8) { const uint2 c2 = *reinterpret_cast<const uint2*>(code + i * E); cw[0] = c2.x; cw[1] = c2.y; }
    else { cw[0] = *reinterpret_cast<const unsigned*>(code + i * E); cw[1] = 0; }
    float g[E];
// ... 148 lines not shown

hipError_t launch_bn_bwd(const BnArgs& a, int is_bf16, hipStream_t st) {
  dim3 grid(a.nchunk, a.G);
  if (is_bf16) hipLaunchKernelGGL((bn_reduce_kernel<bf16, 1>), grid, dim3(256), 0, st, a);
  else hipLaunchKernelGGL((bn_reduce_kernel<float, 1>), grid, dim3(256), 0, st, a);
  hipLaunchKernelGGL(bn_bwd_finalize_kernel, dim3((a.C + 3) / 4), dim3(256), 0, st, a);
  const size_t work = (size_t)a.G * a.Pg * (a.C / (is_bf16 ? 8 : 4));
  VP_DISPATCH(is_bf16, bn_bwd_apply_kernel, dim3(nblocks(work)), dim3(256), st, a);
  return hipGetLastError();
}

hipError_t launch_bn_bwd_tail(const BnArgs& a, int is_bf16, hipStream_t st) {
  hipLaunchKernelGGL(bn_bwd_finalize_kernel, dim3((a.C + 3) / 4), dim3(256), 0, st, a);
  const size_t work = (size_t)a.G * a.Pg * (a.C / (is_bf16 ? 8 : 4));
  VP_DISPATCH(is_bf16, bn_bwd_apply_kernel, dim3(nblocks(work)), dim3(256), st, a);
  return hipGetLastError();
}

__global__ __launch_bounds__(256) void colsum_finalize_kernel(const BnArgs a, int creal, float* out, int accumulate) {
  const int c = blockIdx.x * 4 + (threadIdx.x >> 6), lane = threadIdx.x & 63;
  if (c >= creal) return;
  double s = 0;
  for (int grp = 0; grp < a.G; ++grp) {
    double s0, s1;
    chunk_sum(a, grp, c, lane, s0, s1);
    s += s0;
  }
  if (lane == 0) out[c] = (float)s + (accumulate ? out[c] : 0.f);
}

hipError_t launch_colsum(const BnArgs& a, int creal, float* out, int accumulate, int is_bf16, hipStream_t st) {
  dim3 grid(a.nchunk, a.G);
  if (is_bf16) hipLaunchKernelGGL((bn_reduce_kernel<bf16, 0>), grid, dim3(256), 0, st, a);
  else hipLaunchKernelGGL((bn_reduce_kernel<float, 0>), grid, dim3(256), 0, st, a);
  hipLaunchKernelGGL(colsum_finalize_kernel, dim3((creal + 3) / 4), dim3(256), 0, st, a, creal, out, accumulate);
  return hipGetLastError();
}

hipError_t launch_colsum_tail(const BnArgs& a, int creal, float* out, int accumulate, hipStream_t st) {
  hipLaunchKernelGGL(colsum_finalize_kernel, dim3((creal + 3) / 4), dim3(256), 0, st, a, creal, out, accumulate);
  return hipGetLastError();
}

hipError_t launch_act_apply(const void* y, const float* sc, const float* sh, int C, int Pg, size_t npix,
                            void* out_lrelu, void* out_relu, int is_bf16, hipStream_t st) {
  const size_t work = npix * (C / (is_bf16 ? 8 : 4));
  if (is_bf16) hipLaunchKernelGGL((act_apply_kernel<bf16>), dim3(nblocks(work)), dim3(256), 0, st, (const bf16*)y, sc, sh, C, Pg, npix, (bf16*)out_lrelu, (bf16*)out_relu);
  else hipLaunchKernelGGL((act_apply_kernel<float>), dim3(nblocks(work)), dim3(256), 0, st, (const float*)y, sc, sh, C, Pg, npix, (float*)out_lrelu, (float*)out_relu);
  return hipGetLastError();
}

hipError_t launch_tap_gather(const TapArgs& a, hipStream_t st) {
  hipLaunchKernelGGL(tap_gather_kernel, dim3((unsigned)(((size_t)a.N * a.Hout * a.Wout + 255) / 256)), dim3(256), 0, st, a);
  return hipGetLastError();
}

hipError_t launch_tap_spread(const TapArgs& a, int is_bf16, hipStream_t st) {
  VP_DISPATCH(is_bf16, tap_spread_kernel, dim3((unsigned)(((size_t)a.N * a.Hin * a.Win + 255) / 256)), dim3(256), st, a);
  return hipGetLastError();
}

hipError_t launch_pack_inputs(const PackInputsArgs& a, int is_bf16, hipStream_t st) {
  VP_DISPATCH(is_bf16, pack_inputs_kernel, dim3(nblocks((size_t)a.N * a.HW)), dim3(256), st, a);
  return hipGetLastError();
}

hipError_t launch_frame_pack(const FramePackArgs& a, hipStream_t st) {
  hipLaunchKernelGGL(frame_pack_kernel, dim3(nblocks((size_t)a.N * a.S * a.S * 2)), dim3(256), 0, st, a);
  return hipGetLastError();
}

int composite_nblocks(int N, int HW) { return nblocks((size_t)N * HW, 1024); }

hipError_t launch_composite_fwd(const CompositeArgs& a, int is_bf16, hipStream_t st) {
  VP_DISPATCH(is_bf16, composite_fwd_kernel, dim3(composite_nblocks(a.N, a.HW)), dim3(256), st, a);
  return hipGetLastError();
}

hipError_t launch_composite_bwd(const CompositeArgs& a, int is_bf16, hipStream_t st) {
  VP_DISPATCH(is_bf16, composite_bwd_kernel, dim3(nblocks((size_t)a.N * a.HW)), dim3(256), st, a);
  return hipGetLastError();
}

hipError_t launch_gan_loss(const GanLossArgs& a, int is_bf16, hipStream_t st) {
  VP_DISPATCH(is_bf16, gan_loss_kernel, dim3(1), dim3(1024), st, a);
  return hipGetLastError();
}

int perceptual_nblocks(size_t half, int is_bf16) { return nblocks(half / (is_bf16 ? 8 : 4), 1024); }

hipError_t launch_perceptual(const PerceptualArgs& a, int is_bf16, hipStream_t st) {
  VP_DISPATCH(is_bf16, perceptual_kernel, dim3(perceptual_nblocks(a.half, is_bf16)), dim3(256), st, a);
  return hipGetLastError();
}

hipError_t launch_loss_final(const LossFinalArgs& a, hipStream_t st) {
  hipLaunchKernelGGL(loss_final_kernel, dim3(1), dim3(256), 0, st, a);
  return hipGetLastError();
}

hipError_t launch_maxpool_fwd(const void* x, void* y, int B, int H, int W, int C, int is_bf16, hipStream_t st) {
  const size_t work = (size_t)B * (H / 2) * (W / 2) * (C / (is_bf16 ? 8 : 4));
  if (is_bf16) hipLaunchKernelGGL((maxpool_fwd_kernel<bf16>), dim3(nblocks(work)), dim3(256), 0, st, (const bf16*)x, (bf16*)y, B, H, W, C);
  else hipLaunchKernelGGL((maxpool_fwd_kernel<float>), dim3(nblocks(work)), dim3(256), 0, st, (const float*)x, (float*)y, B, H, W, C);
  return hipGetLastError();
}

hipError_t launch_maxpool_bwd(const void* x, const void* dy, void* dx, int B, int H, int W, int C, int is_bf16, hipStream_t st) {
  const size_t work = (size_t)B * (H / 2) * (W / 2) * (C / (is_bf16 ? 8 : 4));
  if (is_bf16) hipLaunchKernelGGL((maxpool_bwd_kernel<bf16>), dim3(nblocks(work)), dim3(256), 0, st, (const bf16*)x, (const bf16*)dy, (bf16*)dx, B, H, W, C);
  else hipLaunchKernelGGL((maxpool_bwd_kernel<float>), dim3(nblocks(work)), dim3(256), 0, st, (const float*)x, (const float*)dy, (float*)dx, B, H, W, C);
  return hipGetLastError();
}

hipError_t launch_maxpool_bwd_code(const void* code, const void* dy, void* dx, int B, int H, int W, int C, int is_bf16, hipStream_t st) {
  const size_t work = (size_t)B * (H / 2) * (W / 2) * (C / (is_bf16 ? 8 : 4));
  if (is_bf16) hipLaunchKernelGGL((maxpool_bwd_code_kernel<bf16>), dim3(nblocks(work)), dim3(256), 0, st, (const unsigned char*)code, (const bf16*)dy, (bf16*)dx, B, H, W, C);
  else hipLaunchKernelGGL((maxpool_bwd_code_kernel<float>), dim3(nblocks(work)), dim3(256), 0, st, (const unsigned char*)code, (const float*)dy, (float*)dx, B, H, W, C);
  return hipGetLastError();
}

hipError_t launch_relu_bwd(const void* y, void* d, size_t n, int is_bf16, hipStream_t st) {
  const size_t nvec = n / (is_bf16 ? 8 : 4);
  if (is_bf16) hipLaunchKernelGGL((relu_bwd_kernel<bf16>), dim3(nblocks(nvec)), dim3(256), 0, st, (const bf16*)y, (bf16*)d, nvec);
  else hipLaunchKernelGGL((relu_bwd_kernel<float>), dim3(nblocks(nvec)), dim3(256), 0, st, (const float*)y, (float*)d, nvec);
  return hipGetLastError();
}

hipError_t launch_grad_pack_bf16(const float* src, void* dst, size_t n, hipStream_t st) {
  hipLaunchKernelGGL(grad_pack_bf16_kernel, dim3(nblocks(n / 8 + 1, 4096)), dim3(256), 0, st, src, (bf16*)dst, n / 8, n);
  return hipGetLastError();
}

hipError_t launch_grad_unpack_bf16(const void* src, float* dst, size_t n, float scale, hipStream_t st) {
  hipLaunchKernelGGL(grad_unpack_bf16_kernel, dim3(nblocks(n / 8 + 1, 4096)), dim3(256), 0, st, (const bf16*)src, dst, n / 8, n, scale);
  return hipGetLastError();
}

hipError_t launch_adam(const AdamArgs& a, hipStream_t st) {
  hipLaunchKernelGGL(adam_tf_kernel, dim3(nblocks(a.n, 4096)), dim3(256), 0, st, a);
  return hipGetLastError();
}

}
```

voicepuppet_amd/csrc/pointwise_args.h:

```cpp
#pragma once
#include <stddef.h>
#include <stdint.h>

namespace vp {

struct PackDesc {
  size_t src_off;
  size_t dst_off;
  int nclass, rows_real, rows_pad, ntaps, C, C_real, Kpad;
  int kc;
  int perm;
  int kswap;
  int s_kh, s_kw, s_row, s_ch;
  int8_t kh[4][16];
  int8_t kw[4][16];
};

struct FetchArgs {
  const float* raw3;
  const float* fg3;
  const float* o4;
  void* dst;
  size_t npix;
  int mode;
};

struct BnArgs {
  const void* y;
  const void* dz;
  void* dy;
  int C, G, Pg;
  int nchunk;
  double* partial;
  const float* gamma;
  const float* beta;
  float* aff_a;
  float* aff_b;
  float* mu;
  float* rstd;
  float* c1;
  float* c2;
  float* dgamma;
  float* dbeta;
  int accumulate;
  float eps;
  float* dbias_zero;
  int raw;
};

struct PackInputsArgs {
  const float* inputs;
  const float* fg_inputs;
  void* gin;
  void* gfg;
  void* din;
  void* vin;
  int N, HW, train;
  int fg_c;
};

struct FramePackArgs {
  const unsigned char* ex;
  const unsigned char* cur;
  const int* crops;
  float* inputs;
  float* fg_inputs;
  float* targets;
  float* masks;
  int N, S;
};

struct CompositeArgs {
  const float* y4;
  const float* targets;
  const float* masks;
  float* o4;
  float* outputs;
  float* outputs_fg;
  void* din;
  void* vin;
  double* partial;
  int N, HW, train;
  const void* d_din;
  const void* d_vin;
  void* dy4;
  float l1_weight;
};

struct GanLossArgs {
  const float* logits;
  void* dl_d;
  void* dl_g;
  float* predict;
  float* losses;
  int M;
  float gan_weight;
};

struct PerceptualArgs {
  const void* f3;
  void* df3;
  double* partial;
  size_t half;
  float l1_weight;
};

struct LossFinalArgs {
  const double* comp_partial; int n_comp;
  const double* perc_partial; int n_perc;
  double n_out;
  double n_feat;
  float* losses;
  float l1_weight, gan_weight;
};

struct TapArgs {
  const float* S;
  const float* bias;
  float* y;
  const void* dy;
  void* dyS;
  int N, Hin, Win, Hout, Wout, ks, pad, ld_dy;
};

struct AdamArgs {
  float* p; const float* g; float* m; float* v;
  size_t n;
  float lr_t, beta1, beta2, eps;
};

}
```

Measured before the change: 4558 frames/s.

## Fuse perceptual loss into conv3_3 epilogue and parallelize GAN loss reduction

```diff
diff --git a/voicepuppet_amd/csrc/conv_args.h b/voicepuppet_amd/csrc/conv_args.h
--- a/voicepuppet_amd/csrc/conv_args.h
+++ b/voicepuppet_amd/csrc/conv_args.h
@@ -90,6 +90,10 @@
   unsigned* sp_cnt;
   unsigned short sp_mask[4];
   int sp_npt, sp_lcpt;
+  const void* perc_ref;
+  void* perc_dz;
+  double* perc_partial;
+  float perc_s;
 };
 
 struct WgradArgs {
diff --git a/voicepuppet_amd/csrc/conv_ops.h b/voicepuppet_amd/csrc/conv_ops.h
--- a/voicepuppet_amd/csrc/conv_ops.h
+++ b/voicepuppet_amd/csrc/conv_ops.h
@@ -116,6 +116,7 @@
 inline int& patch4_knob() { static int v = 1; return v; }
 inline int& c64_knob() { static int v = 1; return v; }
 inline int& pool_bwd_fused_knob() { static int v = 1; return v; }
+inline int& perceptual_fused_knob() { static int v = 1; return v; }
 inline int& cout1_knob() { static int v = 256; return v; }
 inline int& wgrad1_rows_knob() { static int v = 512; return v; }
 inline int& dc64_knob() { static int v = 1; return v; }
diff --git a/voicepuppet_amd/csrc/conv_patch3.hip b/voicepuppet_amd/csrc/conv_patch3.hip
--- a/voicepuppet_amd/csrc/conv_patch3.hip
+++ b/voicepuppet_amd/csrc/conv_patch3.hip
@@ -18,7 +18,7 @@
 template <typename T, int WC, int WP, int TC, int TP, int TH, int TW, int NSTW, int KW>
 using Patch3Geom = PatchGeom<T, WC, WP, TC, TP, TH, TW, KW - 1, NSTW>;
 
-template <typename T, int WC, int WP, int TC, int TP, int TH, int TW, int STATS, int OCC, int NSTW = 3, int KW = 3>
+template <typename T, int WC, int WP, int TC, int TP, int TH, int TW, int STATS, int OCC, int NSTW = 3, int KW = 3, int PERC = 0>
 __global__ __launch_bounds__(512, OCC) void igemm_patch3_kernel(const IgemmArgs a) {
   using G = Patch3Geom<T, WC, WP, TC, TP, TH, TW, NSTW, KW>;
   constexpr int E = G::E, KC = G::KC, NW = G::NW, LA = NSTW - 1;
@@ -122,11 +122,11 @@
   asm volatile("s_waitcnt vmcnt(0)" ::: "memory");
 
 #ifndef VP_P3_NO_FASTEPI
-  constexpr int NPASS16 = G::BC == 64 ? epi_passes16(G::BC, G::BP, WP, G::RINGB) : 0;
+  constexpr int NPASS16 = (G::BC == 64 || PERC != 0) ? epi_passes16(G::BC, G::BP, WP, G::RINGB) : 0;
 #else
   constexpr int NPASS16 = 0;
 #endif
-  if (!(VP_P3_ABL & 8) || acc[0][0][0] == 1.2345f) staged_epilogue<T, TC, TP, G::BC, G::BP, G::NPASS, G::NT, STATS, NPASS16>(a, PatchTilePix<TW>{a, n, y0, x0}, c_base, blkA0, blkB0, acc, smem, tile.bt, 0);
+  if (!(VP_P3_ABL & 8) || acc[0][0][0] == 1.2345f) staged_epilogue<T, TC, TP, G::BC, G::BP, G::NPASS, G::NT, STATS, NPASS16, false, PERC>(a, PatchTilePix<TW>{a, n, y0, x0}, c_base, blkA0, blkB0, acc, smem, tile.bt, 0);
 }
 
 template <typename T, int WC, int WP, int TC, int TP, int TH, int TW, int OCC, int NSTW = 3, int KW = 3>
@@ -156,10 +156,20 @@
   return launch_patch3_t<bf16, 2, 4, 4, 4, 16, 16, 4, 4, 4>(b, st);
 }
 
+bool patch3_perc_eligible(const IgemmArgs& a, int is_bf16, int bc, int bp) {
+  return is_bf16 && a.kern == CK_PATCH3 && patch3_eligible(a, is_bf16) && bc == 256 && bp == 128 && a.splitk == 1 && !a.ref && !a.accumulate && !a.y_f32 &&
+         (a.out_act == ACT_NONE || a.out_act == ACT_RELU) && !a.bn_part && !a.bst_y && !a.pool_out && a.Cout % 8 == 0 && a.ldY % 8 == 0;
+}
+int patch3_perc_blocks(const IgemmArgs& a) { return a.N * ((a.Hg + 7) / 8) * ((a.Wg + 15) / 16) * (a.CoutPad / 256); }
+
 hipError_t launch_igemm_patch3(const IgemmArgs& a, int is_bf16, int bc, int bp, hipStream_t st) {
   IgemmArgs b = a;
   b.vec_epi = 1;
   b.xcd_remap = patch_xcd_knob();
+  if (a.perc_ref) {
+    if (!patch3_perc_eligible(a, is_bf16, bc, bp) || !a.perc_dz || !a.perc_partial) return hipErrorInvalidValue;
+    return launch_patch_grid<Patch3Geom<bf16, 2, 4, 8, 2, 8, 16, 3, 3>>(igemm_patch3_kernel<bf16, 2, 4, 8, 2, 8, 16, 0, 4, 3, 3, 1>, b, 1, st);
+  }
 #define VP_PATCH3_GO(WC, WP, TC, TP, TH, TW, OCC) \
   (is_bf16 ? launch_patch3_t<bf16, WC, WP, TC, TP, TH, TW, OCC>(b, st) : launch_patch3_t<float, WC, WP, TC, TP, TH, TW, OCC>(b, st))
 #define VP_PATCH3_GO6(WC, WP, TC, TP, TH, TW, OCC) \
diff --git a/voicepuppet_amd/csrc/igemm_device.h b/voicepuppet_amd/csrc/igemm_device.h
--- a/voicepuppet_amd/csrc/igemm_device.h
+++ b/voicepuppet_amd/csrc/igemm_device.h
@@ -137,11 +137,13 @@
   return m > 0.f ? 1u + best : 0u;
 }
 
-template <typename T, int TC, int TP, int BC, int BP, int NPASS, int NT, int STATS = 0, int NPASS16 = 0, bool DUAL = false, typename PixFn>
+template <typename T, int TC, int TP, int BC, int BP, int NPASS, int NT, int STATS = 0, int NPASS16 = 0, bool DUAL = false, int PERC = 0, typename PixFn>
 __device__ __forceinline__ void staged_epilogue(const IgemmArgs& a, const PixFn& pixfn, int c_base, int blkA0, int blkB0,
                                                 f32x4 (&acc)[TC][TP], char* smem, int pt = 0, int cls = 0) {
+  static_assert(PERC == 0 || (NPASS16 > 0 && sizeof(T) == 2 && STATS == 0), "the perceptual epilogue is a form of the bf16-staged path");
   if constexpr (NPASS16 > 0 && sizeof(T) == 2 && STATS == 0) {
-    if (!a.ref && !a.accumulate && !a.y_f32 && (a.out_act == ACT_NONE || a.out_act == ACT_RELU)) {
+    if (PERC != 0 || (!a.ref && !a.accumulate && !a.y_f32 && (a.out_act == ACT_NONE || a.out_act == ACT_RELU))) {
+      [[maybe_unused]] double psum = 0;
       constexpr int PITCHB = BC * 2 + 16, CGB = BC / 8, RPB = BP / NPASS16;
       static_assert(RPB % (TP * 16) == 0, "a wave's pixel rows must fall into one pass");
       const int tid = threadIdx.x, lane = tid & 63;
@@ -179,6 +181,37 @@
         __syncthreads();
         bool store_y = true;
         if constexpr (pix_has_pool<PixFn>::value) store_y = !(a.pool_out != nullptr && a.pool_only);
+        if constexpr (PERC != 0) {
+          store_y = false;
+          constexpr int NIT = (RPB * CGB + NT - 1) / NT;
+          uint4 rk[NIT];
+#pragma unroll
+          for (int it = 0; it < NIT; ++it) {
+            const int idx = tid + it * NT, p = idx / CGB, cgp = idx - p * CGB;
+            const long long ot = idx < RPB * CGB ? otab[p] : -1;
+            const int c0 = c_base + cgp * 8;
+            rk[it] = make_uint4(0, 0, 0, 0);
+            if (ot >= 0 && c0 < a.Cout) rk[it] = *reinterpret_cast<const uint4*>(reinterpret_cast<const bf16*>(a.perc_ref) + (size_t)(ot >> 8) + c0);
+          }
+#pragma unroll
+          for (int it = 0; it < NIT; ++it) {
+            const int idx = tid + it * NT, p = idx / CGB, cgp = idx - p * CGB;
+            const long long ot = idx < RPB * CGB ? otab[p] : -1;
+            const int c0 = c_base + cgp * 8;
+            if (ot < 0 || c0 >= a.Cout) continue;
+            const uint4 pk = *reinterpret_cast<const uint4*>(smem + p * PITCHB + cgp * 16);
+            float fa[8], fb[8], d[8];
+            Elem<bf16>::unpack(rk[it], fa);
+            Elem<bf16>::unpack(pk, fb);
+#pragma unroll
+            for (int e = 0; e < 8; ++e) {
+              const float x = fa[e] - fb[e];
+              psum += (double)x * x;
+              d[e] = (fb[e] > 0.f) ? -a.perc_s * x : 0.f;
+            }
+            *reinterpret_cast<uint4*>(reinterpret_cast<bf16*>(a.perc_dz) + (size_t)(ot >> 8) + c0) = Elem<bf16>::pack(d);
+          }
+        }
         if (store_y)
           for (int idx = tid; idx < RPB * CGB; idx += NT) {
             const int p = idx / CGB, cgp = idx - p * CGB;
@@ -227,6 +260,18 @@
               }
             }
           }
+        }
+      }
+      if constexpr (PERC != 0) {
+        psum = wave_sum(psum);
+        __syncthreads();
+        double* red = reinterpret_cast<double*>(smem);
+        if (lane == 0) red[tid >> 6] = psum;
+        __syncthreads();
+        if (tid == 0) {
+          double s = 0;
+          for (int w = 0; w < NT / 64; ++w) s += red[w];
+          a.perc_partial[blockIdx.x + gridDim.x * blockIdx.y] = s;
         }
       }
       return;
diff --git a/voicepuppet_amd/csrc/launch.h b/voicepuppet_amd/csrc/launch.h
--- a/voicepuppet_amd/csrc/launch.h
+++ b/voicepuppet_amd/csrc/launch.h
@@ -10,6 +10,8 @@
 void igemm_tile(int cfg, int* bc, int* bp);
 hipError_t launch_igemm_patch(const IgemmArgs& a, int is_bf16, int bc, int bp, hipStream_t st);
 bool patch3_eligible(const IgemmArgs& a, int is_bf16);
+bool patch3_perc_eligible(const IgemmArgs& a, int is_bf16, int bc, int bp);
+int patch3_perc_blocks(const IgemmArgs& a);
 hipError_t launch_igemm_patch3(const IgemmArgs& a, int is_bf16, int bc, int bp, hipStream_t st);
 bool patch4_eligible(const IgemmArgs& a, int is_bf16);
 hipError_t launch_igemm_patch4(const IgemmArgs& a, hipStream_t st);
@@ -77,7 +79,9 @@
 int composite_nblocks(int N, int HW);
 hipError_t launch_composite_fwd(const CompositeArgs& a, int is_bf16, hipStream_t st);
 hipError_t launch_composite_bwd(const CompositeArgs& a, int is_bf16, hipStream_t st);
+int gan_loss_nblocks(int m);
 hipError_t launch_gan_loss(const GanLossArgs& a, int is_bf16, hipStream_t st);
+hipError_t launch_gan_loss_final(const GanLossArgs& a, hipStream_t st);
 int perceptual_nblocks(size_t half, int is_bf16);
 hipError_t launch_perceptual(const PerceptualArgs& a, int is_bf16, hipStream_t st);
 hipError_t launch_loss_final(const LossFinalArgs& a, hipStream_t st);
diff --git a/voicepuppet_amd/csrc/ops_api.hip b/voicepuppet_amd/csrc/ops_api.hip
--- a/voicepuppet_amd/csrc/ops_api.hip
+++ b/voicepuppet_amd/csrc/ops_api.hip
@@ -1,6 +1,9 @@
 #include <string.h>
 
+#include <map>
+#include <mutex>
 #include <string>
+#include <utility>
 
 #include "conv_ops.h"
 #include "errors.h"
@@ -66,6 +69,7 @@
   if (k == "c64") { c64_knob() = value; return VP_OK; }
   if (k == "dc64") { dc64_knob() = value; return VP_OK; }
   if (k == "pool_bwd_fused") { pool_bwd_fused_knob() = value < 0 || value > 4 ? 1 : value; return VP_OK; }
+  if (k == "perceptual_fused") { perceptual_fused_knob() = value != 0; return VP_OK; }
   if (k == "cout1_wgrad_rows" && value > 0) { wgrad1_rows_knob() = value; return VP_OK; }
   if (k == "cout1_bwd") { cout1_knob() = value < 0 ? 256 : value; return VP_OK; }
   if (k == "s2c64") { s2c64_knob() = value; return VP_OK; }
@@ -325,7 +329,22 @@
   GanLossArgs ga;
   memset(&ga, 0, sizeof(ga));
   ga.logits = logits; ga.dl_d = seed_d; ga.dl_g = seed_g; ga.predict = predict; ga.losses = losses; ga.M = m; ga.gan_weight = gan_weight;
+  {
+    static std::mutex mu;
+    static std::map<void*, std::pair<double*, int>> tables;
+    std::lock_guard<std::mutex> lk(mu);
+    std::pair<double*, int>& t = tables[stream];
+    const int nb = gan_loss_nblocks(m);
+    if (t.second < nb) {
+      if (t.first) (void)hipFree(t.first);
+      t = {nullptr, 0};
+      VP_HIP_CHECK(hipMalloc((void**)&t.first, (size_t)nb * 2 * sizeof(double)));
+      t.second = nb;
+    }
+    ga.partial = t.first;
+  }
   VP_HIP_CHECK(launch_gan_loss(ga, dtype == VP_BF16, (hipStream_t)stream));
+  VP_HIP_CHECK(launch_gan_loss_final(ga, (hipStream_t)stream));
   return VP_OK;
 }
 
diff --git a/voicepuppet_amd/csrc/plan_pixrefer.hip b/voicepuppet_amd/csrc/plan_pixrefer.hip
--- a/voicepuppet_amd/csrc/plan_pixrefer.hip
+++ b/voicepuppet_amd/csrc/plan_pixrefer.hip
@@ -1,3 +1,4 @@
+#include <algorithm>
 #include <math.h>
 #include <stdio.h>
 #include <string.h>
@@ -133,7 +134,10 @@
   bool pool_fuse_ok[2];
   bool pool_bwd_fused;
   bool pool_dz_stale[2];
-  double *comp_partial, *perc_partial, *bn_partial;
+  bool perc_fuse_ok;
+  int n_perc_fused;
+  bool perc_fused;
+  double *comp_partial, *perc_partial, *gan_partial, *bn_partial;
   char* scratch;
   char* scratch2;
   double* bn_partial2;
@@ -533,7 +537,8 @@
     h->n_comp = composite_nblocks(N, H * H);
     h->n_perc = perceptual_nblocks((size_t)N * (H / 4) * (H / 4) * 256, h->bf16);
     h->comp_partial = (double*)ar.alloc((size_t)h->n_comp * 2 * sizeof(double));
-    h->perc_partial = (double*)ar.alloc((size_t)h->n_perc * sizeof(double));
+    h->perc_partial = (double*)ar.alloc((size_t)std::max(h->n_perc, h->n_perc_fused) * sizeof(double));
+    h->gan_partial = (double*)ar.alloc((size_t)gan_loss_nblocks((int)M) * 2 * sizeof(double));
   }
   h->zeros = ar.alloc(256);
   h->bn_partial = (double*)ar.alloc((size_t)1024 * 2 * 512 * sizeof(double));
@@ -577,6 +582,13 @@
       const bool big = !k || (long long)ba.N * (ba.Hg / 4) * (ba.Wg / 16) >= 4096;
       h->pool_fuse_ok[k] = ((knob == 1 && big) || knob == 2 + k || knob == 4) && h->bf16 && conv_kernel_ok(pool_fused_view(L.bwd_alt[0]), h->bf16);
     }
+    const Layer& L3 = h->V.l.back();
+    if (perceptual_fused_knob() && h->bf16 && L3.scope == "conv3/conv3_3" && L3.has_fwd_half) {
+      int bc, bp;
+      igemm_tile(L3.fwd_half.cfg, &bc, &bp);
+      h->perc_fuse_ok = patch3_perc_eligible(L3.fwd_half.a, h->bf16, bc, bp);
+      if (h->perc_fuse_ok) h->n_perc_fused = patch3_perc_blocks(L3.fwd_half.a);
+    }
   }
   h->scratch_bytes = smax + 256;
   h->params_dirty = true;
@@ -665,8 +677,9 @@
 }
 
 static int run_layer_fwd_half(vp_pixrefer* h, Net& n, Layer& L, int half, hipStream_t st, void* pool_out = nullptr, bool pool_only = false,
-                              unsigned char* pool_code = nullptr) {
+                              unsigned char* pool_code = nullptr, const PerceptualArgs* perc = nullptr) {
   IgemmArgs a = L.fwd_half.a;
+  if (perc) { a.perc_ref = perc->f3; a.perc_dz = perc->df3; a.perc_partial = perc->partial; a.perc_s = perc->l1_weight / (float)perc->half; }
   a.pool_out = pool_out;
   a.pool_only = pool_out && pool_only ? 1 : 0;
   a.pool_code = a.pool_only ? pool_code : nullptr;
@@ -1200,6 +1213,17 @@
       region_of(tp.dz, tp.elems() / 2 * es, (tp.name + ".dz (pooled-source read)").c_str());
       region_of(h->vpool_code[k], tp.elems() / 2, (tp.name + " codes (pooled-source read)").c_str());
     }
+    region_of(h->comp_partial, (size_t)h->n_comp * 2 * sizeof(double), "comp_partial");
+    region_of(h->gan_partial, (size_t)gan_loss_nblocks((int)M) * 2 * sizeof(double), "gan_partial");
+    region_of(h->perc_partial, (size_t)h->n_perc * sizeof(double), "perc_partial");
+    if (h->perc_fuse_ok) {
+      const Layer& L3 = h->V.l.back();
+      int bc, bp;
+      igemm_tile(L3.fwd_half.cfg, &bc, &bp);
+      if (L3.scope != "conv3/conv3_3" || !L3.has_fwd_half || !patch3_perc_eligible(L3.fwd_half.a, h->bf16, bc, bp)) fail("%s fwd_half: no perceptual-loss form of kernel %s", L3.scope.c_str(), conv_kernel_name(L3.fwd_half.a.kern));
+      if (h->n_perc_fused != patch3_perc_blocks(L3.fwd_half.a)) fail("%s fwd_half: %d rows of perceptual sums for %d blocks", L3.scope.c_str(), h->n_perc_fused, patch3_perc_blocks(L3.fwd_half.a));
+      region_of(h->perc_partial, (size_t)h->n_perc_fused * sizeof(double), "perc_partial (conv3_3 epilogue)");
+    }
     region_of(h->scratch2, h->scratch_bytes, "scratch2"); region_of(h->scratch3, h->scratch_bytes, "scratch3");
     region_of(h->scratch4, h->scratch_bytes, "scratch4"); region_of(h->bn_partial4, (size_t)1024 * 2 * 512 * 8, "bn_partial4");
     region_of(h->bn_partial2, (size_t)1024 * 2 * 512 * 8, "bn_partial2"); region_of(h->bn_partial3, (size_t)1024 * 2 * 512 * 8, "bn_partial3");
@@ -1411,7 +1435,7 @@
   const int hd = H / 8 - 2;
   GanLossArgs ga;
   memset(&ga, 0, sizeof(ga));
-  ga.logits = h->logits; ga.dl_d = h->dl_d; ga.dl_g = h->dl_g; ga.predict = h->predict; ga.losses = h->losses;
+  ga.logits = h->logits; ga.dl_d = h->dl_d; ga.dl_g = h->dl_g; ga.predict = h->predict; ga.losses = h->losses; ga.partial = h->gan_partial;
   ga.M = N * hd * hd; ga.gan_weight = d.gan_weight;
   VP_HIP_CHECK(launch_gan_loss(ga, bf, sd));
   if (split_d) VP_HIP_CHECK(hipEventRecord(h->ev_bjoin, h->branch));
@@ -1421,6 +1445,12 @@
   for (Layer& L : V.l)
     if (L.scope == "conv1/conv1_2" || L.scope == "conv2/conv2_2") codes = codes && plan_can_pool(L.fwd_half);
   h->pool_codes_written = codes;
+  const Tens& f3 = V.t.back();
+  PerceptualArgs pa;
+  memset(&pa, 0, sizeof(pa));
+  pa.f3 = f3.y; pa.df3 = f3.dz; pa.partial = h->perc_partial; pa.half = f3.elems() / 2; pa.l1_weight = d.l1_weight;
+  const bool perc_fused = split_vgg && bf && !h->store_first_raw && h->perc_fuse_ok;
+  h->perc_fused = perc_fused;
   auto vgg_half = [&](int half, hipStream_t s2) -> int {
     for (size_t i = 0; i < V.l.size(); ++i) {
       Layer& L = V.l[i];
@@ -1431,14 +1461,17 @@
       Tens& tp = V.t[pooled ? L.out + 1 : L.out];
       const size_t oi = (size_t)half * N * ti.H * ti.W * ti.C * h->es, op = (size_t)half * N * tp.H * tp.W * tp.C * h->es;
       const bool code = fuse && codes && half == 1;
-      if ((rc2 = run_layer_fwd_half(h, V, L, half, s2, fuse ? (char*)tp.y + op : nullptr, code, code ? h->vpool_code[L.scope == "conv2/conv2_2"] : nullptr))) return rc2;
+      const bool perc = perc_fused && half == 1 && i + 1 == V.l.size();
+      if (perc) VP_HIP_CHECK(hipStreamWaitEvent(s2, h->ev_join, 0));
+      if ((rc2 = run_layer_fwd_half(h, V, L, half, s2, fuse ? (char*)tp.y + op : nullptr, code, code ? h->vpool_code[L.scope == "conv2/conv2_2"] : nullptr,
+                                    perc ? &pa : nullptr))) return rc2;
       if (pooled && !fuse) VP_HIP_CHECK(launch_maxpool_fwd((const char*)ti.y + oi, (char*)tp.y + op, N, ti.H, ti.W, ti.C, bf, s2));
     }
     return VP_OK;
   };
   if (split_vgg) {
     if ((rc = vgg_half(1, st))) return rc;
-    VP_HIP_CHECK(hipStreamWaitEvent(st, h->ev_join, 0));
+    if (!perc_fused) VP_HIP_CHECK(hipStreamWaitEvent(st, h->ev_join, 0));
   } else {
     for (size_t i = 0; i < V.l.size(); ++i) {
       Layer& L = V.l[i];
@@ -1452,16 +1485,13 @@
       }
     }
   }
-  const Tens& f3 = V.t.back();
-  PerceptualArgs pa;
-  memset(&pa, 0, sizeof(pa));
-  pa.f3 = f3.y; pa.df3 = f3.dz; pa.partial = h->perc_partial; pa.half = f3.elems() / 2; pa.l1_weight = d.l1_weight;
-  VP_HIP_CHECK(launch_perceptual(pa, bf, st));
+  if (!perc_fused) VP_HIP_CHECK(launch_perceptual(pa, bf, st));
 
   if (split_d) VP_HIP_CHECK(hipStreamWaitEvent(st, h->ev_bjoin, 0));
   LossFinalArgs lf;
   memset(&lf, 0, sizeof(lf));
-  lf.comp_partial = h->comp_partial; lf.n_comp = h->n_comp; lf.perc_partial = h->perc_partial; lf.n_perc = h->n_perc;
+  lf.comp_partial = h->comp_partial; lf.n_comp = h->n_comp; lf.perc_partial = h->perc_partial; lf.n_perc = perc_fused ? h->n_perc_fused : h->n_perc;
+  lf.gan_partial = h->gan_partial; lf.n_gan = gan_loss_nblocks(ga.M); lf.gan_M = ga.M;
   lf.n_out = (double)N * H * H * 3; lf.n_feat = (double)pa.half; lf.losses = h->losses;
   lf.l1_weight = d.l1_weight; lf.gan_weight = d.gan_weight;
   VP_HIP_CHECK(launch_loss_final(lf, st));
@@ -1605,6 +1635,7 @@
   if (std::string(key) == "bwd_sums_launches") return h->bst_count;
   if (std::string(key) == "pool_codes_written") return h->pool_codes_written ? 1 : 0;
   if (std::string(key) == "pool_bwd_fused") return h->pool_bwd_fused ? 1 : 0;
+  if (std::string(key) == "perceptual_fused") return h->perc_fused ? 1 : 0;
   return -1;
 }
 
@@ -1842,6 +1873,10 @@
       set_err("vp_pixrefer_tensor: the full-resolution output of %s is not stored (the step keeps its 2x2 max pool and the pool's arg-max codes); vp_pixrefer_set_option(h, \"store_first_raw\", 1) before the forward pass", s.c_str());
       return VP_ERR_STATE;
     }
+    if (field.empty() && n == &h->V && h->perc_fused && t.name == "conv3/conv3_3") {
+      set_err("vp_pixrefer_tensor: the fake half of %s is not stored (its launch takes the perceptual loss and stores the loss's seed); vp_pixrefer_set_option(h, \"store_first_raw\", 1) before the forward pass", s.c_str());
+      return VP_ERR_STATE;
+    }
     if (field.empty()) return ret(t.y, t.N, t.H, t.W, t.is_f32 ? (t.name == "decoder_1" ? 4 : 1) : t.C, (t.is_f32 || t.hi) ? VP_F32 : cd);
     if (field == "dz32") return t.hi ? ret(t.dz32, t.N, t.H, t.W, t.C, VP_F32) : VP_ERR_ARG;
     if (field == "dy" && n == &h->V && (t.name == "conv1/conv1_2" || t.name == "conv2/conv2_2") && h->pool_dz_stale[t.name == "conv2/conv2_2"]) {
diff --git a/voicepuppet_amd/csrc/pointwise.hip b/voicepuppet_amd/csrc/pointwise.hip
--- a/voicepuppet_amd/csrc/pointwise.hip
+++ b/voicepuppet_amd/csrc/pointwise.hip
@@ -644,13 +644,14 @@
 }
 
 template <typename T>
-__global__ __launch_bounds__(1024) void gan_loss_kernel(const GanLossArgs a) {
+__global__ __launch_bounds__(256) void gan_loss_kernel(const GanLossArgs a) {
   const float eps = 1e-12f;
   double acc[2] = {0, 0};
   const float invM = 1.f / (float)a.M;
   T* dld = reinterpret_cast<T*>(a.dl_d);
   T* dlg = reinterpret_cast<T*>(a.dl_g);
-  for (int i = threadIdx.x; i < a.M; i += 1024) {
+  const int i = blockIdx.x * 256 + threadIdx.x;
+  if (i < a.M) {
     const float p0 = 1.f / (1.f + expf(-a.logits[i]));
     const float p1 = 1.f / (1.f + expf(-a.logits[a.M + i]));
     const float pf = 1.f / (1.f + expf(-a.logits[2 * a.M + i]));
@@ -667,7 +668,19 @@
   }
   __shared__ double sm[64];
   block_sum<2>(acc, sm);
-  if (threadIdx.x == 0) { a.losses[0] = (float)(acc[0] / a.M); a.losses[1] = (float)(acc[1] / a.M); }
+  if (threadIdx.x == 0) { a.partial[2 * blockIdx.x] = acc[0]; a.partial[2 * blockIdx.x + 1] = acc[1]; }
+}
+
+__device__ __forceinline__ void gan_partial_rows(const double* partial, int n, double& s0, double& s1) {
+  for (int i = threadIdx.x; i < n; i += 256) { s0 += partial[2 * i]; s1 += partial[2 * i + 1]; }
+}
+
+__global__ __launch_bounds__(256) void gan_loss_final_kernel(const GanLossArgs a, int n) {
+  double v[2] = {0, 0};
+  gan_partial_rows(a.partial, n, v[0], v[1]);
+  __shared__ double sm[64];
+  block_sum<2>(v, sm);
+  if (threadIdx.x == 0) { a.losses[0] = (float)(v[0] / a.M); a.losses[1] = (float)(v[1] / a.M); }
 }
 
 template <typename T>
@@ -696,12 +709,14 @@
 }
 
 __global__ __launch_bounds__(256) void loss_final_kernel(const LossFinalArgs a) {
-  double v[3] = {0, 0, 0};
+  double v[5] = {0, 0, 0, 0, 0};
   for (int i = threadIdx.x; i < a.n_comp; i += 256) { v[0] += a.comp_partial[2 * i]; v[1] += a.comp_partial[2 * i + 1]; }
   for (int i = threadIdx.x; i < a.n_perc; i += 256) v[2] += a.perc_partial[i];
-  __shared__ double sm[64];
-  block_sum<3>(v, sm);
+  gan_partial_rows(a.gan_partial, a.n_gan, v[3], v[4]);
+  __shared__ double sm[80];
+  block_sum<5>(v, sm);
   if (threadIdx.x != 0) return;
+  a.losses[0] = (float)(v[3] / a.gan_M); a.losses[1] = (float)(v[4] / a.gan_M);
   const double content = v[2] / 2.0 / a.n_feat;
   const double gl1 = v[0] / a.n_out + v[1] / a.n_out + content;
   a.losses[2] = (float)gl1;
@@ -1016,8 +1031,15 @@
   return hipGetLastError();
 }
 
+int gan_loss_nblocks(int m) { return (m + 255) / 256; }
+
 hipError_t launch_gan_loss(const GanLossArgs& a, int is_bf16, hipStream_t st) {
-  VP_DISPATCH(is_bf16, gan_loss_kernel, dim3(1), dim3(1024), st, a);
+  VP_DISPATCH(is_bf16, gan_loss_kernel, dim3(gan_loss_nblocks(a.M)), dim3(256), st, a);
+  return hipGetLastError();
+}
+
+hipError_t launch_gan_loss_final(const GanLossArgs& a, hipStream_t st) {
+  hipLaunchKernelGGL(gan_loss_final_kernel, dim3(1), dim3(256), 0, st, a, gan_loss_nblocks(a.M));
   return hipGetLastError();
 }
 
diff --git a/voicepuppet_amd/csrc/pointwise_args.h b/voicepuppet_amd/csrc/pointwise_args.h
--- a/voicepuppet_amd/csrc/pointwise_args.h
+++ b/voicepuppet_amd/csrc/pointwise_args.h
@@ -93,6 +93,7 @@
   void* dl_g;
   float* predict;
   float* losses;
+  double* partial;
   int M;
   float gan_weight;
 };
@@ -110,6 +111,8 @@
   const double* perc_partial; int n_perc;
   double n_out;
   double n_feat;
+  const double* gan_partial; int n_gan;
+  int gan_M;
   float* losses;
   float l1_weight, gan_weight;
 };
```

Result: no change. 4577 frames/s, median of 2 (+0.4%).
